# teofum/platinum

Measured on AMD Instinct MI355X. Metric: Msamples/s (paths x spp x bounces / s) at 1920x1080, 8 bounces, higher is better.
Workload: dtype f32; 1 GPU; C3 1.04M-triangle instanced sphere field, 1920x1080; width=1920, height=1080, max_bounces=8, samples_in_flight=128, spp_per_gpu=1792, spp_total=1792, integrator=MIS+NEE, flags=MultiscatterGGX, triangles=1036300, call_pattern=render(spp_per_step) per step, batches=14, nonfinite_policy=zero (a NaN/inf sample counts as black; parity default is propagate), parallelism=sample-sharded x1, one process per GPU + RCCL all-reduce

## Files before the change

### platinum_amd/csrc/kernels.hip

```cpp
#include <hip/hip_runtime.h>

#include "kernels.h"
#include "pt_denoise.h"
#include "pt_post.h"
#include "pt_shade.h"
#include "queue_plan.h"

namespace pt {

__device__ __forceinline__ vec4 ld_stream(const vec4* p) {
  using f4 = __attribute__((ext_vector_type(4))) float;
  const f4 v = __builtin_nontemporal_load((const f4*)p);
  return vec4{v.x, v.y, v.z, v.w};
}
__device__ __forceinline__ uint32_t ld_stream(const uint32_t* p) { return __builtin_nontemporal_load(p); }
__device__ __forceinline__ void st_stream(vec4* p, vec4 v) {
  using f4 = __attribute__((ext_vector_type(4))) float;
  __builtin_nontemporal_store(f4{v.x, v.y, v.z, v.w}, (f4*)p);
}
__device__ __forceinline__ void st_stream(uint32_t* p, uint32_t v) { __builtin_nontemporal_store(v, p); }

__device__ __forceinline__ uint32_t wave_prefix(unsigned long long mask) {
  return __builtin_amdgcn_mbcnt_hi((uint32_t)(mask >> 32), __builtin_amdgcn_mbcnt_lo((uint32_t)mask, 0u));
}
__device__ __forceinline__ uint32_t wave_sum(uint32_t v) {
  for (int off = 32; off > 0; off >>= 1) v += __shfl_xor(v, off, 64);
  return v;
}
__device__ __forceinline__ uint32_t wave_index() { return blockIdx.x * (blockDim.x >> 6) + (threadIdx.x >> 6); }
__device__ __forceinline__ uint32_t wave_count() { return gridDim.x * (blockDim.x >> 6); }
#ifdef PT_TAIL_PROBE
#define PT_TAIL_BEGIN const unsigned long long tail_t0 = wall_clock64(); unsigned long long tail_take = 0, tail_setup = 0, tail_ta = 0;
#define PT_TAIL_T(acc) { const unsigned long long tb_ = wall_clock64(); acc += tb_ - tail_ta; tail_ta = tb_; }
#define PT_TAIL_MARK tail_ta = wall_clock64();
#define PT_TAIL_END(kind)                                                                                         \
  if (wave_lane() == 0 && bounce < 16u) {                                                                           \
    const unsigned long long t1 = wall_clock64();                                                                   \
    atomicMax(&ctr->tail_end_max[kind][bounce], t1); atomicAdd(&ctr->tail_end_sum[kind][bounce], t1);              \
    atomicMax(&ctr->tail_start_inv[kind][bounce], ~tail_t0); atomicAdd(&ctr->tail_waves[kind][bounce], 1ull);     \
    atomicAdd(&ctr->tail_take[kind][bounce], tail_take); atomicAdd(&ctr->tail_setup[kind][bounce], tail_setup);     \
    atomicAdd(&ctr->tail_busy[kind][bounce], t1 - tail_t0);                                                         \
  }
#else
#define PT_TAIL_BEGIN
#define PT_TAIL_END(kind)
#define PT_TAIL_T(acc)
#define PT_TAIL_MARK
#endif

constexpr uint32_t kClaimMax = 8;

__device__ __forceinline__ uint32_t chunk_entry(uint32_t sg, uint32_t k, uint32_t rays) { return ((rays - 1u) << 26) | (k << 16) | sg; }
static_assert(kMaxSegments <= 65536 && kMaxSegmentSlots / 64 <= 1024, "chunk_entry packs 16 + 10 + 6 bits");

struct ChunkClaims {
  const uint32_t* __restrict__ table;
  uint32_t* cursor;
  uint32_t nseg, total, lane;
  uint32_t next_c, end_c, run_c = 0;
  uint32_t e0 = 0, e1 = 0, e2 = 0, e3 = 0, e4 = 0, e5 = 0, e6 = 0, e7 = 0;
  uint32_t claim_k = kClaimMax, nwaves_grid = 1;
  __device__ __forceinline__ void init(const uint32_t* tab, uint32_t total_, uint32_t* cur, const Segments& seg, uint32_t lane_) {
    table = tab; total = total_; cursor = cur; nseg = seg.nseg; lane = lane_;
    next_c = end_c = 0;
    nwaves_grid = gridDim.x * (blockDim.x >> 6);
    claim_k = guided(total);
  }
  __device__ __forceinline__ uint32_t guided(uint32_t remaining) const {
    return remaining > 32u * nwaves_grid ? kClaimMax : remaining > 8u * nwaves_grid ? 4u : remaining > 2u * nwaves_grid ? 2u : 1u;
  }
  uint32_t pool_next = 0, pool_end = 0;
  bool exhausted = false;
  __device__ __forceinline__ uint32_t take(bool need) {
    uint32_t got = kInvalidRef;
    for (;;) {
      const unsigned long long m = __ballot(need && got == kInvalidRef);
      if (m == 0) return got;
      if (pool_next == pool_end) {
        if (exhausted) return got;
        if (next_c == end_c) {
          uint32_t base = 0;
          if (lane == 0) base = atomicAdd(cursor, claim_k);
          base = __builtin_amdgcn_readfirstlane(base);
          if (base >= total) { exhausted = true; return got; }
          next_c = run_c = base;
          end_c = base + claim_k < total ? base + claim_k : total;
          claim_k = guided(total - end_c);
          const int ev = (int)table[base + (lane & 7u)];
          e0 = (uint32_t)__builtin_amdgcn_readlane(ev, 0); e1 = (uint32_t)__builtin_amdgcn_readlane(ev, 1); e2 = (uint32_t)__builtin_amdgcn_readlane(ev, 2);
          e3 = (uint32_t)__builtin_amdgcn_readlane(ev, 3); e4 = (uint32_t)__builtin_amdgcn_readlane(ev, 4); e5 = (uint32_t)__builtin_amdgcn_readlane(ev, 5);
          e6 = (uint32_t)__builtin_amdgcn_readlane(ev, 6); e7 = (uint32_t)__builtin_amdgcn_readlane(ev, 7);
        }
        const uint32_t at = next_c++ - run_c;
        const uint32_t e = at == 0u ? e0 : at == 1u ? e1 : at == 2u ? e2 : at == 3u ? e3 : at == 4u ? e4 : at == 5u ? e5 : at == 6u ? e6 : e7;
        pool_next = seg_slot(nseg, e & 0xffffu, ((e >> 16) & 0x3ffu) * 64u);
        pool_end = pool_next + (e >> 26) + 1u;
      }
      if (need && got == kInvalidRef) {
        const uint32_t idx = pool_next + wave_prefix(m);
        if (idx < pool_end) got = idx;
      }
      const uint32_t avail = pool_end - pool_next, want = (uint32_t)__popcll(m);
      pool_next += want < avail ? want : avail;
    }
  }
};

constexpr uint32_t kTableBlocks = 32;
__global__ void __launch_bounds__(1024) k_chunk_tables(Segments seg, uint32_t cur, BatchCounters* __restrict__ ctr,
                                                        uint32_t bounce_closest, uint32_t bounce_shadow, uint32_t do_shadow) {
  if (blockIdx.y == 2) {
    if (blockIdx.x != 0) return;
    const uint32_t* __restrict__ cnt = seg.active[cur];
    const uint32_t* __restrict__ cost = seg.shade_cost + (size_t)bounce_closest * seg.nseg;
    __shared__ uint32_t hist[256];
    if (threadIdx.x < 256) hist[threadIdx.x] = 0;
    __syncthreads();
    auto size_class = [&](uint32_t w) {
      const uint32_t c = cost[w], v = c ? c : cnt[w];
      const uint32_t e = 31u - (uint32_t)__builtin_clz(v | 8u);
      return 255u - (v < 8u ? v : (e - 2u) * 8u + ((v >> (e - 3u)) & 7u));
    };
    for (uint32_t w = threadIdx.x; w < seg.nseg; w += 1024) atomicAdd(&hist[size_class(w)], 1u);
    __syncthreads();
    if (threadIdx.x == 0) { uint32_t run = 0; for (int b = 0; b < 256; b++) { const uint32_t h = hist[b]; hist[b] = run; run += h; } }
    __syncthreads();
    for (uint32_t w = threadIdx.x; w < seg.nseg; w += 1024) seg.shade_order[atomicAdd(&hist[size_class(w)], 1u)] = w;
    return;
  }
  const bool sh = blockIdx.y == 1;
  if (sh && !do_shadow) return;
  const uint32_t* __restrict__ counts = sh ? seg.shadow : seg.active[cur];
  uint32_t* __restrict__ table = sh ? seg.table_shadow : seg.table_closest;
  __shared__ uint32_t part[1024];
  __shared__ uint32_t base_sh;
  const uint32_t slice = (seg.nseg + kTableBlocks - 1) / kTableBlocks;
  const uint32_t w_begin = blockIdx.x * slice;
  const uint32_t w_end = w_begin + slice < seg.nseg ? w_begin + slice : seg.nseg;
  uint32_t before = 0, total = 0;
  for (uint32_t w = threadIdx.x; w < seg.nseg; w += 1024) {
    const uint32_t nc = (counts[w] + 63u) / 64u;
    total += nc;
    if (w < w_begin) before += nc;
  }
  part[threadIdx.x] = before;
  __syncthreads();
  for (uint32_t off = 512; off > 0; off >>= 1) { if (threadIdx.x < off) part[threadIdx.x] += part[threadIdx.x + off]; __syncthreads(); }
  if (threadIdx.x == 0) base_sh = part[0];
  __syncthreads();
  if (blockIdx.x == kTableBlocks - 1) {
    part[threadIdx.x] = total;
    __syncthreads();
    for (uint32_t off = 512; off > 0; off >>= 1) { if (threadIdx.x < off) part[threadIdx.x] += part[threadIdx.x + off]; __syncthreads(); }
    if (threadIdx.x == 0) {
      if (sh) ctr->chunks_shadow[bounce_shadow] = part[0];
      else ctr->chunks_closest[bounce_closest] = part[0];
    }
    __syncthreads();
  }
  __shared__ uint32_t rays_of[1024];
  const uint32_t mine_n = (w_begin + threadIdx.x < w_end) ? counts[w_begin + threadIdx.x] : 0u;
  rays_of[threadIdx.x] = mine_n;
  const uint32_t mine = (mine_n + 63u) / 64u;
  part[threadIdx.x] = mine;
  __syncthreads();
  for (uint32_t off = 1; off < 1024; off <<= 1) {
    const uint32_t v = threadIdx.x >= off ? part[threadIdx.x - off] : 0;
    __syncthreads();
    part[threadIdx.x] += v;
    __syncthreads();
  }
  const uint32_t n_entries = part[1023];
  const uint32_t base = base_sh;
  for (uint32_t e = threadIdx.x; e < n_entries; e += 1024) {
    uint32_t lo = 0, hi = 1023;
    while (lo < hi) { const uint32_t mid = (lo + hi) >> 1; if (part[mid] > e) hi = mid; else lo = mid + 1; }
    const uint32_t k = e - (lo ? part[lo - 1] : 0u);
    const uint32_t left = rays_of[lo] - k * 64u;
    table[base + e] = chunk_entry(w_begin + lo, k, left < 64u ? left : 64u);
  }
}

__global__ void __launch_bounds__(kBlock) k_raygen(DeviceScene S, PathState st, vec4* __restrict__ Lbuf, Segments seg,
                                                    BatchCounters* __restrict__ ctr, uint32_t first_sample,
                                                    uint32_t nsamples, uint32_t tilesX, uint32_t tilesY) {
  const uint32_t lane = wave_lane();
  const uint32_t tiles = tilesX * tilesY;
  uint32_t started = 0;
  for (uint32_t sg = wave_index(); sg < seg.nseg; sg += wave_count()) {
    uint32_t n_out = 0;
    const uint32_t first_tile = segment_first_tile(seg, sg);
    for (uint32_t k = 0; k < seg.tiles_per_seg * nsamples; k++) {
      const uint32_t tile = first_tile + k / nsamples;
      if (tile >= tiles) break;
      const uint32_t r = (k % nsamples) * 64u + lane;
      const uint32_t pl = r / nsamples, s = r - pl * nsamples;
      const PixelXY q = tile_pixel(tile, pl, tilesX);
      const bool valid = q.x < S.width && q.y < S.height;
      RayGenOut rg;
      if (valid) rg = stage_raygen(S, q.x, q.y, first_sample + s);
      const unsigned long long m = __ballot(valid);
      if (valid) {
        const uint32_t j = seg_slot(seg.nseg, sg, n_out + wave_prefix(m));
        const uint32_t pid = lbuf_index(tile, s, nsamples, pl);
        const uint32_t rel = pid - first_tile * nsamples * 64u;
        st.rayO[j] = vec4{rg.o.x, rg.o.y, rg.o.z, 0.0f};
        st.rayD[j] = vec4{rg.d.x, rg.d.y, rg.d.z, u2f((rg.dim & kMetaDimMask) | (rel << kMetaPidShift))};
        st.att[j] = vec4{1.0f, 1.0f, 1.0f, u2f(rg.offset)};
        Lbuf[pid] = vec4{0.0f, 0.0f, 0.0f, 1.0f};
      }
      n_out += (uint32_t)__popcll(m);
    }
    if (lane == 0) { seg.active[0][sg] = n_out; seg.poison[sg] = 0u; }
    started += n_out;
  }
  if (lane == 0) {
    WaveStats& ws = seg.stats[wave_index()];
    ws.paths += started;
    ws.closest += started;
  }
}

__global__ void __launch_bounds__(kBlock) k_raygen_adaptive(DeviceScene S, PathState st, vec4* __restrict__ Lbuf, Segments seg,
                                                             uint32_t first_sample, uint32_t nsamples, uint32_t tilesX, Rect rect,
                                                             const uint32_t* __restrict__ active, const uint32_t* __restrict__ active_count) {
  const uint32_t lane = wave_lane();
  const uint32_t tiles = *active_count;
  uint32_t started = 0;
  for (uint32_t sg = wave_index(); sg < seg.nseg; sg += wave_count()) {
    uint32_t n_out = 0;
    const uint32_t first_tile = segment_first_tile(seg, sg);
    for (uint32_t k = 0; k < seg.tiles_per_seg * nsamples; k++) {
      const uint32_t tile = first_tile + k / nsamples;
      if (tile >= tiles) break;
      const uint32_t r = (k % nsamples) * 64u + lane;
      const uint32_t pl = r / nsamples, s = r - pl * nsamples;
      const PixelXY q = tile_pixel(active[tile], pl, tilesX);
      const bool valid = rect_contains(rect, q.x, q.y);
      RayGenOut rg;
      if (valid) rg = stage_raygen(S, q.x, q.y, first_sample + s);
      const unsigned long long m = __ballot(valid);
      if (valid) {
        const uint32_t j = seg_slot(seg.nseg, sg, n_out + wave_prefix(m));
        const uint32_t pid = lbuf_index(tile, s, nsamples, pl);
        const uint32_t rel = pid - first_tile * nsamples * 64u;
        st.rayO[j] = vec4{rg.o.x, rg.o.y, rg.o.z, 0.0f};
        st.rayD[j] = vec4{rg.d.x, rg.d.y, rg.d.z, u2f((rg.dim & kMetaDimMask) | (rel << kMetaPidShift))};
        st.att[j] = vec4{1.0f, 1.0f, 1.0f, u2f(rg.offset)};
        Lbuf[pid] = vec4{0.0f, 0.0f, 0.0f, 1.0f};
      }
      n_out += (uint32_t)__popcll(m);
    }
    if (lane == 0) { seg.active[0][sg] = n_out; seg.poison[sg] = 0u; }
    started += n_out;
  }
  if (lane == 0) {
    WaveStats& ws = seg.stats[wave_index()];
    ws.paths += started;
    ws.closest += started;
  }
}

#ifndef PT_TWO_BLOCK
#define PT_TWO_BLOCK 1024
#define PT_TWO_BLOCKS_PER_CU 1
#define PT_TWO_LDS_NODES 1024
#endif
constexpr uint32_t kTraceBlock2 = PT_TWO_BLOCK;
constexpr uint32_t kLdsNodes = PT_TWO_LDS_NODES;
#ifndef PT_TRI_VOTE
#define PT_TRI_VOTE 2
#endif
template <bool ANY, bool COUNT, bool TWO, bool W6 = false>
__device__ __forceinline__ void wave_traverse(const DeviceScene& S, const BvhNode* lds_nodes, TravState& ts, TraversalCount* tc) {
  constexpr int kRoom = W6 ? 1 : 4, kRows = W6 ? kPendLeaves6 : kPendLeaves;
  if (ts.cur != kInvalidRef && ts.st.npend <= kRows - kRoom) {
    if (TWO) {
      trav_leave(ts);
      const bool at_inst = ts.cur != kInvalidRef && (ts.cur & kInstBit) != 0;
      const bool at_node = ts.cur != kInvalidRef && !at_inst;
      const unsigned long long mi = __ballot(at_inst), mn = __ballot(at_node);
      if (mi != 0 && (2 * __popcll(mi) >= __popcll(mn) || mn == 0)) {
        if (at_inst) trav_resolve(S, ts);
      } else if (at_node) {
        if (lds_nodes) trav_node<COUNT, true>(lds_nodes, ts, tc); else trav_node<COUNT, true>(S.nodes, ts, tc);
      }
    } else if (W6) {
      trav_node6<COUNT>(S.nodes, ts, tc);
    } else {
      trav_node<COUNT, false>(S.nodes, ts, tc);
    }
  }
  const bool pending = ts.st.npend > 0;
  const bool stuck = pending && (ts.cur == kInvalidRef || ts.st.npend > kRows - kRoom);
  const bool advancing = ts.cur != kInvalidRef && !stuck;
  const unsigned long long mp = __ballot(pending);
  if (mp == 0) return;
  const bool go = PT_TRI_VOTE * __popcll(mp) >= __popcll(__ballot(1)) || __ballot(ts.st.npend > kRows - kRoom) != 0 || __ballot(advancing) == 0;
  if (go && pending) {
    const bool fin = W6 ? trav_pending_leaf6<ANY, COUNT>(S, ts, tc) : trav_pending_leaf<ANY, COUNT>(S, ts, tc);
    if (fin) { ts.cur = kInvalidRef; ts.st.npend = 0; ts.st.sp = 0; }
  }
}

__device__ __forceinline__ const BvhNode* stage_nodes(const DeviceScene& S, BvhNode* lds_nodes) {
  if (S.node_count > kLdsNodes) return nullptr;
  const uint4* src = reinterpret_cast<const uint4*>(S.nodes);
  uint4* dst = reinterpret_cast<uint4*>(lds_nodes);
  for (uint32_t i = threadIdx.x; i < S.node_count * 4; i += blockDim.x) dst[i] = src[i];
  __syncthreads();
  return lds_nodes;
}

template <bool COUNT, bool TWO, bool W6 = false>
__global__ void __launch_bounds__(TWO ? kTraceBlock2 : kBlock, TWO ? PT_TWO_BLOCKS_PER_CU : PT_CLOSEST_WAVES)
k_trace_closest(DeviceScene S, PathState st, vec4* __restrict__ hit, Segments seg, uint32_t cur, BatchCounters* __restrict__ ctr, uint32_t bounce,
                uint32_t* __restrict__ spill, int32_t* __restrict__ hitlog, uint32_t log_stride) {
  PT_TAIL_BEGIN
  constexpr uint32_t kTB = TWO ? kTraceBlock2 : kBlock;
  __shared__ uint32_t lds_stack[(W6 ? kLdsStack6 : kLdsStack) + 1][kTB];
  __shared__ uint32_t lds_pend[(W6 ? kPendLeaves6 : kPendLeaves) + 1][kTB];
  __shared__ BvhNode lds_nodes_buf[TWO && kLdsNodes ? kLdsNodes : 1];
  const BvhNode* lds_nodes = TWO && kLdsNodes ? stage_nodes(S, lds_nodes_buf) : nullptr;
  const uint32_t lane = wave_lane();
  ChunkClaims src;
  src.init(seg.table_closest, ctr->chunks_closest[bounce], &ctr->work_closest[bounce], seg, lane);
  TraversalStack stack;
  stack.lds = &lds_stack[0][threadIdx.x];
  stack.pend = &lds_pend[0][threadIdx.x];
  stack.lds_stride = kTB;
  stack.spill = spill + ((size_t)blockIdx.x * kTB + threadIdx.x);
  stack.spill_stride = gridDim.x * kTB;
  TraversalCount tc;

  TravState ts;
  uint32_t ray = kInvalidRef;
  auto finish = [&]() {
    const RayHit& h = ts.best;
#ifdef PT_DEBUG_PID
    if (ts.dbg) printf("dbg finish: t %.9g u %.9g v %.9g tri %u gid %u\n", h.t, h.u, h.v, h.tri, h.gid >> 2);
    ts.dbg = false;
#endif
    hit[ray] = vec4{h.t, h.u, h.v, u2f(h.tri == kInvalidRef ? kInvalidRef : (h.tri | ((h.gid & 3u) << 28)))};
    if (hitlog) {
      const uint32_t pixel = pixel_of_pid_1spp(segment_lbuf_base(seg, slot_segment(seg.nseg, ray)) + (f2u(st.rayD[ray].w) >> kMetaPidShift), S.width);
      int32_t* hl = &hitlog[((size_t)bounce * log_stride + pixel) * 2];
      hl[0] = hl[1] = -1;
      if (h.tri != kInvalidRef) triangle_ids(S, h.tri, &hl[0], &hl[1]);
    }
    ray = kInvalidRef;
  };
  const uint32_t refill = seg.refill_threshold;
  for (;;) {
    PT_TAIL_MARK
    const uint32_t fresh = src.take(ray == kInvalidRef);
    PT_TAIL_T(tail_take)
    if (fresh != kInvalidRef) {
      ray = fresh;
      const vec4 o4 = st.rayO[ray];
      const vec4 d4 = st.rayD[ray];
      float ir = 0.0f;
      if (S.has_alpha) ir = Halton{halton_table(S.halton), f2u(st.att[ray].w), f2u(d4.w) & kMetaDimMask}.sample1d();
#ifdef PT_DEBUG_PID
      ts.dbg = ctr->_pad[1] == bounce + 1u && segment_lbuf_base(seg, slot_segment(seg.nseg, ray)) + (f2u(d4.w) >> kMetaPidShift) == ctr->_pad[0];
      if (ts.dbg) printf("dbg ray slot %u lane %u wave %u o %.9g %.9g %.9g d %.9g %.9g %.9g\n", ray, lane, wave_index(), o4.x, o4.y, o4.z, d4.x, d4.y, d4.z);
#endif
      if (trav_init(S, ts, v3(o4.x, o4.y, o4.z), v3(d4.x, d4.y, d4.z), 1e-3f, kInf, ir, stack, false, COUNT ? &tc : nullptr)) finish();
    }
    PT_TAIL_T(tail_setup)
    if (__ballot(ray != kInvalidRef) == 0) {
      if (src.exhausted && src.pool_next == src.pool_end) break;
      continue;
    }
    while (ray != kInvalidRef) {
      wave_traverse<false, COUNT, TWO, W6>(S, lds_nodes, ts, &tc);
      if (ts.cur == kInvalidRef && ts.st.npend == 0) finish();
      if (refill && !src.exhausted && (uint32_t)__popcll(__ballot(ray != kInvalidRef)) < refill) break;
    }
  }
  if (COUNT) {
    const uint32_t nn = wave_sum(tc.nodes), t = wave_sum(tc.tris);
    if (lane == 0) {
      atomicAdd(&ctr->nodes_closest, (unsigned long long)nn);
      atomicAdd(&ctr->tris_closest, (unsigned long long)t);
    }
  }
  PT_TAIL_END(0)
}

#ifndef PT_SHADE_WAVES
#define PT_SHADE_WAVES 4
#endif
#ifndef PT_SHADE_BLOCK
#define PT_SHADE_BLOCK 256
#endif
constexpr uint32_t kShadeBlock = PT_SHADE_BLOCK;
constexpr uint32_t kShadeHalton = 128;
constexpr uint32_t kShadeLights = 64;
constexpr int kLutE = 128, kLutEavg = 128, kLutEavgMs = 32;
constexpr uint32_t kBinCap = 128;

__global__ void __launch_bounds__(PT_SHADE_BLOCK, (PT_SHADE_WAVES * 4 * 64) / PT_SHADE_BLOCK)
k_shade(const DeviceScene* __restrict__ Sp, PathState sin, PathState sout, const vec4* __restrict__ hit, ShadowQueue sq,
        vec4* __restrict__ Lbuf, Segments seg, uint32_t cur, BatchCounters* __restrict__ ctr, uint32_t bounce) {
  PT_TAIL_BEGIN
  const DeviceScene& S = *Sp;
  __shared__ HaltonEntry lds_halton[kShadeHalton];
  __shared__ LightRec lds_lights[kShadeLights];
  __shared__ float lds_Eavg[kLutEavg];
  __shared__ float lds_EavgMs[kLutEavgMs * kLutEavgMs];
  static_assert(kMaxSegmentSlots <= 65536, "slot numbers inside a segment are binned as uint16_t (queue_plan.h bounds seg_cap)");
  __shared__ uint16_t lds_bins[kShadeBlock / 64][5][kBinCap];
  __shared__ uint32_t lds_bin_tri[kShadeBlock / 64][5][kBinCap];
  const uint32_t halton_base = 5u + 7u * bounce;
  uint32_t halton_count = 11u + 5u * bounce;
  if (halton_base >= (uint32_t)kHaltonDims) halton_count = 0;
  else if (halton_base + halton_count > (uint32_t)kHaltonDims) halton_count = (uint32_t)kHaltonDims - halton_base;
  if (halton_count > kShadeHalton) halton_count = kShadeHalton;
  const bool lights_in_lds = S.lightCount <= kShadeLights;
  {
    const uint4* src = reinterpret_cast<const uint4*>(S.halton + halton_base);
    uint4* dst = reinterpret_cast<uint4*>(lds_halton);
    for (uint32_t i = threadIdx.x; i < halton_count * 2; i += kShadeBlock) dst[i] = ldg(&src[i]);
    if (lights_in_lds) {
      const uint4* ls = reinterpret_cast<const uint4*>(S.light_recs);
      uint4* ld = reinterpret_cast<uint4*>(lds_lights);
      for (uint32_t i = threadIdx.x; i < S.lightCount * (uint32_t)(sizeof(LightRec) / 16); i += kShadeBlock) ld[i] = ldg(&ls[i]);
    }
    for (uint32_t i = threadIdx.x; i < (uint32_t)kLutEavg; i += kShadeBlock) lds_Eavg[i] = ldg(&S.luts.Eavg.d[i]);
    for (uint32_t i = threadIdx.x; i < (uint32_t)(kLutEavgMs * kLutEavgMs); i += kShadeBlock) lds_EavgMs[i] = ldg(&S.luts.EavgMs.d[i]);
  }
  __syncthreads();
  ShadeTables T;
  T.luts.E = Lut{S.luts.E.d, kLutE, kLutE, 1, 0};
  T.luts.Eavg = Lut{lds_Eavg, kLutEavg, 1, 1, 1};
  T.luts.EMs = Lut{S.luts.EMs.d, S.luts.EMs.w, S.luts.EMs.h, S.luts.EMs.depth, 0};
  T.luts.EavgMs = Lut{lds_EavgMs, kLutEavgMs, kLutEavgMs, 1, 1};
  T.luts.ETransIn = Lut{S.luts.ETransIn.d, S.luts.ETransIn.w, S.luts.ETransIn.h, S.luts.ETransIn.depth, 0};
  T.luts.ETransOut = Lut{S.luts.ETransOut.d, S.luts.ETransOut.w, S.luts.ETransOut.h, S.luts.ETransOut.depth, 0};
  T.halton = HaltonTab{S.halton, lds_halton, halton_base, halton_count};
  T.lights = lights_in_lds ? lds_lights : S.light_recs;
  T.light_cdf = S.light_cdf;
  T.lights_lds = lights_in_lds ? 1 : 0;

  const uint32_t lane = wave_lane();
  uint32_t shaded = 0, total_out = 0, total_shadow = 0;
  uint32_t claim = wave_index();
  uint16_t* bin = &lds_bins[threadIdx.x >> 6][0][0];
  uint32_t* bin_tri = &lds_bin_tri[threadIdx.x >> 6][0][0];
  while (claim < seg.nseg) {
    const uint32_t sg = __builtin_amdgcn_readfirstlane(seg.shade_order[claim]);
    const unsigned long long seg_t0 = wall_clock64();
    const uint32_t lbuf_base = segment_lbuf_base(seg, sg);
    const uint32_t n = __builtin_amdgcn_readfirstlane(seg.active[cur][sg]);
    uint32_t n_out = 0, n_shadow = 0;
    const uint32_t seg_poisoned = S.env_texture < 0 ? __builtin_amdgcn_readfirstlane(seg.poison[sg]) : 0u;
    unsigned long long poisoned_now = 0;
    uint32_t cnt0 = 0, cnt1 = 0, cnt2 = 0, cnt3 = 0, cnt4 = 0;
    uint32_t k0 = 0;
    for (;;) {
      while (k0 < n && cnt0 < 64 && cnt1 < 64 && cnt2 < 64 && cnt3 < 64 && cnt4 < 64) {
        const uint32_t k = k0 + lane;
        uint32_t cls = 5;
        uint32_t w = 0;
        if (k < n) {
          w = f2u(hit[seg_slot(seg.nseg, sg, k)].w);
          cls = w == kInvalidRef ? 4u : (w >> 28) & 3u;
          if (w == kInvalidRef && S.env_texture < 0) {
            if (!seg_poisoned) cls = 5u;
            else {
              const vec4 a4 = sin.att[seg_slot(seg.nseg, sg, k)];
              if (!att_poisoned(v3(a4.x, a4.y, a4.z))) cls = 5u;
            }
          }
        }
        const unsigned long long m0 = __ballot(cls == 0), m1 = __ballot(cls == 1), m2 = __ballot(cls == 2), m3 = __ballot(cls == 3),
                                 m4 = __ballot(cls == 4);
        if (cls < 5) {
          const uint32_t at = cls == 0 ? cnt0 + wave_prefix(m0) : cls == 1 ? cnt1 + wave_prefix(m1) : cls == 2 ? cnt2 + wave_prefix(m2)
                            : cls == 3 ? cnt3 + wave_prefix(m3) : cnt4 + wave_prefix(m4);
          bin[cls * kBinCap + at] = (uint16_t)k;
          bin_tri[cls * kBinCap + at] = w & kHitTriMask;
        }
        cnt0 += (uint32_t)__popcll(m0); cnt1 += (uint32_t)__popcll(m1); cnt2 += (uint32_t)__popcll(m2);
        cnt3 += (uint32_t)__popcll(m3); cnt4 += (uint32_t)__popcll(m4);
        k0 += 64;
      }
      uint32_t k = kInvalidRef, tri = 0;
      bool is_miss = false;
      const uint32_t full = cnt0 >= 64 ? 0u : cnt1 >= 64 ? 1u : cnt2 >= 64 ? 2u : cnt3 >= 64 ? 3u : cnt4 >= 64 ? 4u : 5u;
      if (full < 5) {
        uint32_t c = 0;
        if (full == 0) c = cnt0 -= 64; else if (full == 1) c = cnt1 -= 64; else if (full == 2) c = cnt2 -= 64;
        else if (full == 3) c = cnt3 -= 64; else c = cnt4 -= 64;
        k = bin[full * kBinCap + c + lane];
        tri = bin_tri[full * kBinCap + c + lane];
        is_miss = full == 4;
      } else {
        if (cnt0 + cnt1 + cnt2 + cnt3 + cnt4 == 0) break;
        uint32_t taken = 0;
#define PT_TAKE_FROM(c, cnt)                                                                                                   \
        {                                                                                                                      \
          const uint32_t take = cnt < 64 - taken ? cnt : 64 - taken;                                                           \
          if (lane >= taken && lane < taken + take) { k = bin[c * kBinCap + cnt - take + (lane - taken)]; tri = bin_tri[c * kBinCap + cnt - take + (lane - taken)]; is_miss = c == 4; }  \
          cnt -= take;                                                                                                         \
          taken += take;                                                                                                       \
        }
        PT_TAKE_FROM(0, cnt0) PT_TAKE_FROM(1, cnt1) PT_TAKE_FROM(2, cnt2) PT_TAKE_FROM(3, cnt3) PT_TAKE_FROM(4, cnt4)
#undef PT_TAKE_FROM
      }
      const bool has = k != kInvalidRef && !is_miss;
      const uint32_t i = seg_slot(seg.nseg, sg, k != kInvalidRef ? k : 0u);
      if (k != kInvalidRef && is_miss) {
        const vec4 o4 = sin.rayO[i];
        const vec4 d4 = sin.rayD[i];
        const vec4 a4 = sin.att[i];
        const vec3 att = v3(a4.x, a4.y, a4.z);
        const uint32_t mpid = lbuf_base + (f2u(d4.w) >> kMetaPidShift);
        vec4 L = Lbuf[mpid];
        if (S.env_texture >= 0) {
          const vec3 Le = stage_miss(S, v3(d4.x, d4.y, d4.z), att, bounce, o4.w, (f2u(d4.w) & kMetaSpecular) != 0);
          L.x += Le.x; L.y += Le.y; L.z += Le.z;
        }
        L.x += att.x * 0.0f; L.y += att.y * 0.0f; L.z += att.z * 0.0f;
        Lbuf[mpid] = L;
      }
      uint32_t c_shadow = 0, c_alive = 0;
      if (has) {
        const vec4 h4 = ld_stream(&hit[i]);
        const vec4 o4 = ld_stream(&sin.rayO[i]);
        const vec4 d4 = ld_stream(&sin.rayD[i]);
        const vec4 a4 = ld_stream(&sin.att[i]);
        const uint32_t meta = f2u(d4.w);
        const uint32_t pid = lbuf_base + (meta >> kMetaPidShift);
        ShadeIn in;
        in.o = v3(o4.x, o4.y, o4.z);
        in.d = v3(d4.x, d4.y, d4.z);
        in.att = v3(a4.x, a4.y, a4.z);
        in.rayO = &sin.rayO[i];
        in.rayD = &sin.rayD[i];
        in.lastSpecular = (meta & kMetaSpecular) != 0;
        in.offset = f2u(a4.w);
        in.dim = (meta & kMetaDimMask) + 1;
        in.bounce = bounce;
        in.t = h4.x; in.u = h4.y; in.v = h4.z;
        in.tri = tri;
        ShadeGeom g;
        ShadingContext sc;
        shade_geometry(S, in, g, sc);
        const BSDF bsdf(sc, S.flags, T.luts, g.wo);
        uint32_t dim_rr;
        {
          const NeeOut nee = shade_nee(S, T, in, g, sc, bsdf, in.dim + 6);
          dim_rr = nee.dim;
          const unsigned long long m = __ballot(nee.shadow);
          if (nee.shadow) {
            const uint32_t j = seg_slot(seg.nseg, sg, n_shadow + wave_prefix(m));
            st_stream(&sq.o[j], vec4{g.hitPos.x, g.hitPos.y, g.hitPos.z, nee.tmax});
            st_stream(&sq.d[j], vec4{nee.d.x, nee.d.y, nee.d.z, u2f(pid)});
            st_stream(&sq.contrib[j], vec4{nee.contrib.x, nee.contrib.y, nee.contrib.z, nee.payload});
          }
          c_shadow = (uint32_t)__popcll(m);
        }
        const BounceOut bo = shade_bounce(S, T, in, g, sc, bsdf, dim_rr);
        if (bo.has_emitted) {
          vec4 L = Lbuf[pid];
          L.x += bo.emitted.x; L.y += bo.emitted.y; L.z += bo.emitted.z;
          Lbuf[pid] = L;
        }
        const unsigned long long m = __ballot(bo.alive);
        poisoned_now |= __ballot(bo.alive && att_poisoned(bo.next_att));
        if (bo.alive) {
          const uint32_t j = seg_slot(seg.nseg, sg, n_out + wave_prefix(m));
          st_stream(&sout.rayO[j], vec4{g.hitPos.x, g.hitPos.y, g.hitPos.z, bo.next_pdf});
          st_stream(&sout.rayD[j], vec4{bo.next_d.x, bo.next_d.y, bo.next_d.z, u2f((bo.dim & kMetaDimMask) | (bo.next_specular ? kMetaSpecular : 0u) | (meta & ~(kMetaDimMask | kMetaSpecular)))});
          st_stream(&sout.att[j], vec4{bo.next_att.x, bo.next_att.y, bo.next_att.z, u2f(in.offset)});
        }
        c_alive = (uint32_t)__popcll(m);
      }
      const unsigned long long mh = __ballot(has);
      if (mh) {
        const int src = __builtin_ctzll(mh);
        n_shadow += (uint32_t)__builtin_amdgcn_readlane((int)c_shadow, src);
        n_out += (uint32_t)__builtin_amdgcn_readlane((int)c_alive, src);
        shaded += (uint32_t)__popcll(mh);
      }
    }
    if (lane == 0) {
      seg.active[cur ^ 1][sg] = n_out;
      seg.shadow[sg] = n_shadow;
      if (poisoned_now) seg.poison[sg] = 1u;
      seg.shade_cost[(size_t)bounce * seg.nseg + sg] = (uint32_t)(wall_clock64() - seg_t0) + 1u;
    }
    total_out += n_out;
    total_shadow += n_shadow;
    uint32_t next = 0;
    if (lane == 0) next = wave_count() + atomicAdd(&ctr->work_shade[bounce], 1u);
    claim = __builtin_amdgcn_readfirstlane(next);
  }
  if (lane == 0) {
    WaveStats& ws = seg.stats[wave_index()];
    ws.closest += total_out;
    ws.shadow += total_shadow;
    ws.shaded += shaded;
  }
  PT_TAIL_END(1)
}

template <bool COUNT, bool TWO, bool W6 = false>
__global__ void __launch_bounds__(TWO ? kTraceBlock2 : kBlock, TWO ? PT_TWO_BLOCKS_PER_CU : PT_SHADOW_WAVES)
k_trace_shadow(DeviceScene S, ShadowQueue sq, vec4* __restrict__ Lbuf, Segments seg, BatchCounters* __restrict__ ctr, uint32_t bounce,
               uint32_t* __restrict__ spill) {
  PT_TAIL_BEGIN
  constexpr uint32_t kTB = TWO ? kTraceBlock2 : kBlock;
  __shared__ uint32_t lds_stack[(W6 ? kLdsStack6 : kLdsStack) + 1][kTB];
  __shared__ uint32_t lds_pend[(W6 ? kPendLeaves6 : kPendLeaves) + 1][kTB];
  __shared__ BvhNode lds_nodes_buf[TWO && kLdsNodes ? kLdsNodes : 1];
  const BvhNode* lds_nodes = TWO && kLdsNodes ? stage_nodes(S, lds_nodes_buf) : nullptr;
  const uint32_t lane = wave_lane();
  ChunkClaims src;
  src.init(seg.table_shadow, ctr->chunks_shadow[bounce], &ctr->work_shadow[bounce], seg, lane);
  TraversalStack stack;
  stack.lds = &lds_stack[0][threadIdx.x];
  stack.pend = &lds_pend[0][threadIdx.x];
  stack.lds_stride = kTB;
  stack.spill = spill + ((size_t)blockIdx.x * kTB + threadIdx.x);
  stack.spill_stride = gridDim.x * kTB;
  TraversalCount tc;

  TravState ts;
  uint32_t ray = kInvalidRef, pid = 0;
  auto finish = [&]() {
    if (ts.best.tri == kInvalidRef) {
      const vec4 c = sq.contrib[ray];
      vec4 L = Lbuf[pid];
      L.x += c.x; L.y += c.y; L.z += c.z;
      Lbuf[pid] = L;
    }
    ray = kInvalidRef;
  };
  const uint32_t refill = seg.refill_threshold;
  for (;;) {
    PT_TAIL_MARK
    const uint32_t fresh = src.take(ray == kInvalidRef);
    PT_TAIL_T(tail_take)
    if (fresh != kInvalidRef) {
      ray = fresh;
      const vec4 o4 = sq.o[ray];
      const vec4 d4 = sq.d[ray];
      pid = f2u(d4.w);
      const float ir = S.has_alpha ? sq.contrib[ray].w : 0.0f;
      if (trav_init(S, ts, v3(o4.x, o4.y, o4.z), v3(d4.x, d4.y, d4.z), 1e-3f, o4.w, ir, stack, true, COUNT ? &tc : nullptr)) finish();
    }
    PT_TAIL_T(tail_setup)
    if (__ballot(ray != kInvalidRef) == 0) {
      if (src.exhausted && src.pool_next == src.pool_end) break;
      continue;
    }
    while (ray != kInvalidRef) {
      wave_traverse<true, COUNT, TWO, W6>(S, lds_nodes, ts, &tc);
      if (ts.cur == kInvalidRef && ts.st.npend == 0) finish();
      if (refill && !src.exhausted && (uint32_t)__popcll(__ballot(ray != kInvalidRef)) < refill) break;
    }
  }
  if (COUNT) {
    const uint32_t nn = wave_sum(tc.nodes), t = wave_sum(tc.tris);
    if (lane == 0) {
      atomicAdd(&ctr->nodes_shadow, (unsigned long long)nn);
      atomicAdd(&ctr->tris_shadow, (unsigned long long)t);
    }
  }
  PT_TAIL_END(2)
}

template <bool ADAPTIVE>
__device__ __forceinline__ void accumulate_body(vec4* __restrict__ acc, const vec4* __restrict__ Lbuf, uint32_t npixels, uint32_t width,
                                                uint32_t nsamples, uint32_t n0, uint32_t nonfinite_policy, BatchCounters* __restrict__ ctr,
                                                const uint32_t* __restrict__ active, const uint32_t* __restrict__ active_count,
                                                vec2* __restrict__ mom, uint32_t* __restrict__ tile_n, Rect rect) {
  constexpr uint32_t kRow = 9;
  __shared__ vec4 stage[kBlock / 64][64 * kRow];
  const uint32_t lane = wave_lane(), w = threadIdx.x >> 6;
  const uint32_t height = npixels / width, tilesX = tiles_x(width), tiles = ADAPTIVE ? *active_count : tilesX * tiles_y(height);
  const uint32_t tile = blockIdx.x * (kBlock / 64) + w;
  const bool live = tile < tiles;
  const uint32_t itile = ADAPTIVE ? (live ? active[tile] : 0u) : tile;
  const PixelXY q = tile_pixel(itile, lane, tilesX);
  const bool inside = live && (ADAPTIVE ? rect_contains(rect, q.x, q.y) : q.x < width && q.y < height);
  const uint32_t p = q.y * width + q.x;
  vec4 a = inside ? acc[p] : vec4{0.0f, 0.0f, 0.0f, 0.0f};
  vec2 m = ADAPTIVE && inside && mom ? mom[p] : vec2{0.0f, 0.0f};
  for (uint32_t s0 = 0; s0 < nsamples; s0 += 8u) {
    const uint32_t nb = nsamples - s0 < 8u ? nsamples - s0 : 8u;
    __syncthreads();
    if (live) {
#pragma unroll
      for (uint32_t i = 0; i < 8u; i++) {
        const uint32_t px = i * 8u + (lane >> 3), j = lane & 7u;
        if (j < nb) stage[w][px * kRow + j] = ld_stream(&Lbuf[lbuf_index(tile, s0 + j, nsamples, px)]);
      }
    }
    __syncthreads();
    if (inside) {
      for (uint32_t j = 0; j < nb; j++) {
        const vec4 v = stage[w][lane * kRow + j];
        vec3 L = v3(v.x, v.y, v.z);
        if (!(fabsf(L.x) <= 3.0e38f && fabsf(L.y) <= 3.0e38f && fabsf(L.z) <= 3.0e38f)) {
          atomicAdd(&ctr->nonfinite, 1u);
          if (nonfinite_policy == PT_NONFINITE_ZERO) L = v3(0.0f);
        }
        const uint32_t localFrameIdx = n0 + s0 + j;
        if (ADAPTIVE) {
          const float lum = dn_lum(L);
          m = vec2{aov_fold(m.x, lum, localFrameIdx), aov_fold(m.y, lum * lum, localFrameIdx)};
        }
        if (localFrameIdx > 0) {
          L = L + v3(a.x, a.y, a.z) * (float)localFrameIdx;
          L = L / (float)(localFrameIdx + 1);
        }
        a = vec4{L.x, L.y, L.z, 1.0f};
      }
    }
  }
  if (inside) acc[p] = a;
  if (ADAPTIVE) {
    if (inside && mom) mom[p] = m;
    if (live && lane == 0) tile_n[itile] = n0 + nsamples;
  }
}

__global__ void __launch_bounds__(kBlock) k_accumulate(vec4* __restrict__ acc, const vec4* __restrict__ Lbuf,
                                                        uint32_t npixels, uint32_t width, uint32_t nsamples, uint32_t n0,
                                                        uint32_t nonfinite_policy, BatchCounters* __restrict__ ctr) {
  accumulate_body<false>(acc, Lbuf, npixels, width, nsamples, n0, nonfinite_policy, ctr, nullptr, nullptr, nullptr, nullptr, Rect{});
}

__global__ void __launch_bounds__(kBlock) k_accumulate_adaptive(vec4* __restrict__ acc, const vec4* __restrict__ Lbuf,
                                                                 uint32_t npixels, uint32_t width, uint32_t nsamples, uint32_t n0,
                                                                 uint32_t nonfinite_policy, BatchCounters* __restrict__ ctr,
                                                                 const uint32_t* __restrict__ active, const uint32_t* __restrict__ active_count,
                                                                 vec2* __restrict__ mom, uint32_t* __restrict__ tile_n, Rect rect) {
  accumulate_body<true>(acc, Lbuf, npixels, width, nsamples, n0, nonfinite_policy, ctr, active, active_count, mom, tile_n, rect);
}

__global__ void __launch_bounds__(kBlock) k_accumulate_gmon(vec4* __restrict__ buckets, const vec4* __restrict__ Lbuf,
                                                             uint32_t npixels, uint32_t width, uint32_t nsamples, uint32_t n0,
                                                             uint32_t samples_per_bucket, uint32_t gmon_buckets, uint32_t bucket_base,
                                                             uint32_t nonfinite_policy, BatchCounters* __restrict__ ctr) {
  const uint32_t p = blockIdx.x * kBlock + threadIdx.x;
  if (p >= npixels) return;
  const uint32_t l0 = lbuf_index_of_pixel(p, width, 0, nsamples);
  constexpr uint32_t kGroup = 8u;
  vec4 v[kGroup];
  for (uint32_t s = 0; s < nsamples; s++) {
    if (s % kGroup == 0) {
#pragma unroll
      for (uint32_t j = 0; j < kGroup; j++)
        if (s + j < nsamples) v[j] = ld_stream(&Lbuf[l0 + (s + j)]);
    }
    vec4 L4 = v[0];
#pragma unroll
    for (uint32_t j = 1; j < kGroup; j++) if (s % kGroup == j) L4 = v[j];
    vec3 L = v3(L4.x, L4.y, L4.z);
    if (!(fabsf(L.x) <= 3.0e38f && fabsf(L.y) <= 3.0e38f && fabsf(L.z) <= 3.0e38f)) {
      atomicAdd(&ctr->nonfinite, 1u);
      if (nonfinite_policy == PT_NONFINITE_ZERO) L = v3(0.0f);
    }
    const uint32_t f = n0 + s;
    vec4* acc = buckets + (size_t)(f / samples_per_bucket - bucket_base) * npixels;
    const uint32_t localFrameIdx = f / gmon_buckets;
    if (localFrameIdx > 0) {
      const vec4 a = acc[p];
      L = L + v3(a.x, a.y, a.z) * (float)localFrameIdx;
      L = L / (float)(localFrameIdx + 1);
    }
    acc[p] = vec4{L.x, L.y, L.z, 1.0f};
  }
}

__global__ void __launch_bounds__(kBlock) k_gmon(vec4* __restrict__ acc, const vec4* __restrict__ buckets, uint32_t npixels,
                                                  uint32_t nBuckets, float cap) {
  const uint32_t p = blockIdx.x * kBlock + threadIdx.x;
  if (p >= npixels) return;
  const vec3 lw = v3(0.2126f, 0.7152f, 0.0722f);
  vec3 values[32];
  for (uint32_t i = 0; i < nBuckets; i++) {
    const vec4 b = buckets[(size_t)i * npixels + p];
    values[i] = v3(b.x, b.y, b.z);
  }
  for (uint32_t i = nBuckets; i > 1; i--)
    for (uint32_t j = 1; j < i; j++)
      if (dot(values[j], lw) < dot(values[j - 1], lw)) {
        const vec3 temp = values[j - 1];
        values[j - 1] = values[j];
        values[j] = temp;
      }
  vec3 sum = v3(0.0f), weightedSum = v3(0.0f);
  for (uint32_t i = 0; i < nBuckets; i++) {
    sum = sum + values[i];
    weightedSum = weightedSum + (float)(i + 1) * values[i];
  }
  float G = (2.0f * dot(weightedSum, lw)) / ((float)nBuckets * dot(sum, lw)) - (float)(nBuckets + 1) / (float)nBuckets;
  G = fminf(G, cap);
  const float cf = G * (float)(nBuckets / 2);
  const int c = cf > 0.0f ? (int)cf : 0;
  sum = v3(0.0f);
  for (int i = c; i < (int)nBuckets - c; i++) sum = sum + values[i];
  const vec3 color = sum / (float)((int)nBuckets - 2 * c);
  acc[p] = vec4{color.x, color.y, color.z, 1.0f};
}

__global__ void __launch_bounds__(kBlock) k_weighted_add(vec4* __restrict__ out, const vec4* __restrict__ in, float w, uint32_t npixels,
                                                          uint32_t first, uint32_t last) {
  const uint32_t p = blockIdx.x * kBlock + threadIdx.x;
  if (p >= npixels) return;
  const vec4 a = in[p];
  vec4 o = first ? vec4{0.0f, 0.0f, 0.0f, 0.0f} : out[p];
  o.x += w * a.x; o.y += w * a.y; o.z += w * a.z;
  o.w = last ? 1.0f : 0.0f;
  out[p] = o;
}

__global__ void __launch_bounds__(kBlock) k_postprocess(const vec4* __restrict__ acc, uint32_t* __restrict__ rgba8, uint32_t W,
                                                         uint32_t H, PostConstants pc) {
  const uint32_t p = blockIdx.x * kBlock + threadIdx.x;
  if (p >= W * H) return;
  const uint32_t py = p / W, px = p - py * W;
  rgba8[p] = pp_pack_rgba8(postprocess_pixel(acc, W, H, px, py, pc));
}

__global__ void __launch_bounds__(kBlock) k_fold_counters(const BatchCounters* __restrict__ ctr, Totals* __restrict__ tot,
                                                           Segments seg, uint32_t counted) {
  __shared__ unsigned long long red[4][kBlock];
  unsigned long long a[4] = {0, 0, 0, 0};
  for (uint32_t w = threadIdx.x; w < seg.nstats; w += kBlock) {
    WaveStats& ws = seg.stats[w];
    a[0] += ws.closest; a[1] += ws.shadow; a[2] += ws.shaded; a[3] += ws.paths;
    ws.closest = 0; ws.shadow = 0; ws.shaded = 0; ws.paths = 0;
  }
  for (int k = 0; k < 4; k++) red[k][threadIdx.x] = a[k];
  __syncthreads();
  if (threadIdx.x != 0) return;
  unsigned long long t[4] = {0, 0, 0, 0};
  for (int k = 0; k < 4; k++)
    for (int i = 0; i < kBlock; i++) t[k] += red[k][i];
  if (!counted) {
    tot->closest_rays += t[0];
    tot->shadow_rays += t[1];
    tot->shaded_hits += t[2];
    tot->paths += t[3];
    tot->nonfinite += ctr->nonfinite;
  } else {
    tot->nodes_closest += ctr->nodes_closest; tot->tris_closest += ctr->tris_closest;
    tot->nodes_shadow += ctr->nodes_shadow; tot->tris_shadow += ctr->tris_shadow;
    tot->counted_closest += t[0]; tot->counted_shadow += t[1];
  }
}

__global__ void __launch_bounds__(kBlock) k_light_records(DeviceScene S, LightRec* __restrict__ out, float* __restrict__ cdf) {
  const uint32_t i = blockIdx.x * kBlock + threadIdx.x;
  if (i < S.lightCount) { out[i] = make_light_rec(S, S.lights[i]); cdf[i] = S.lights[i].cumulativePower; }
}

__global__ void __launch_bounds__(kBlock) k_shade_records(DeviceScene S, ShadeRec* __restrict__ out) {
  const uint32_t t = blockIdx.x * kBlock + threadIdx.x;
  if (t >= 2u * S.slot_count) return;
  const TriRec& tr = S.tris[t >> 1];
  const uint32_t gid = (t & 1u) ? tr.gid_b : tr.gid_a;
  if (gid == kInvalidRef) { out[t] = ShadeRec{}; return; }
  const uint32_t inst = tr.inst_code & kSlotInstMask;
  out[t] = make_shade_rec(S, inst, (gid >> 2) - S.instances[inst].tri_global_base);
}

__global__ void __launch_bounds__(kBlock) k_hit_records(DeviceScene S, PathState st, const vec4* __restrict__ hit, Segments seg,
                                                         pt_hit_record* __restrict__ out) {
  const uint32_t lane = wave_lane();
  for (uint32_t sg = wave_index(); sg < seg.nseg; sg += wave_count()) {
    const uint32_t n = seg.active[0][sg];
    for (uint32_t k = lane; k < n; k += 64) {
      const uint32_t i = seg_slot(seg.nseg, sg, k);
      const vec4 h = hit[i];
      const uint32_t tri = f2u(h.w) == kInvalidRef ? kInvalidRef : (f2u(h.w) & kHitTriMask);
      pt_hit_record r;
      if (tri != kInvalidRef) {
        r.t = h.x; r.u = h.y; r.v = h.z;
        triangle_ids(S, tri, &r.instance, &r.primitive);
      } else {
        r.t = 0.0f; r.u = 0.0f; r.v = 0.0f; r.instance = -1; r.primitive = -1;
      }
      out[pixel_of_pid_1spp(segment_lbuf_base(seg, sg) + (f2u(st.rayD[i].w) >> kMetaPidShift), S.width)] = r;
    }
  }
}

void launch_raygen(hipStream_t s, uint32_t grid, const DeviceScene& S, PathState st, vec4* Lbuf, Segments seg, BatchCounters* ctr,
                   uint32_t first_sample, uint32_t nsamples) {
  hipLaunchKernelGGL(k_raygen, dim3(grid), dim3(kBlock), 0, s, S, st, Lbuf, seg, ctr, first_sample, nsamples, tiles_x(S.width), tiles_y(S.height));
}
void launch_raygen_adaptive(hipStream_t s, uint32_t grid, const DeviceScene& S, PathState st, vec4* Lbuf, Segments seg,
                            uint32_t first_sample, uint32_t nsamples, const Rect& rect, const uint32_t* active, const uint32_t* active_count) {
  hipLaunchKernelGGL(k_raygen_adaptive, dim3(grid), dim3(kBlock), 0, s, S, st, Lbuf, seg, first_sample, nsamples, tiles_x(S.width), rect, active,
                     active_count);
}
void launch_chunk_tables(hipStream_t s, Segments seg, uint32_t cur, BatchCounters* ctr, uint32_t bounce_closest,
                         uint32_t bounce_shadow, bool do_shadow) {
  hipLaunchKernelGGL(k_chunk_tables, dim3(kTableBlocks, 3), dim3(1024), 0, s, seg, cur, ctr, bounce_closest, bounce_shadow, do_shadow ? 1u : 0u);
}
uint32_t trace_block_threads(bool two_level) { return two_level ? kTraceBlock2 : (uint32_t)kBlock; }
uint32_t trace_blocks_per_cu_two_level() { return PT_TWO_BLOCKS_PER_CU; }
void launch_trace_closest(hipStream_t s, uint32_t grid, const DeviceScene& S, PathState st, vec4* hit, Segments seg, uint32_t cur,
                          BatchCounters* ctr, uint32_t bounce, uint32_t* spill, int32_t* hitlog, uint32_t log_stride, bool count) {
  if (S.two_level) {
    if (count)
      hipLaunchKernelGGL((k_trace_closest<true, true>), dim3(grid), dim3(kTraceBlock2), 0, s, S, st, hit, seg, cur, ctr, bounce, spill, hitlog, log_stride);
    else
      hipLaunchKernelGGL((k_trace_closest<false, true>), dim3(grid), dim3(kTraceBlock2), 0, s, S, st, hit, seg, cur, ctr, bounce, spill, hitlog, log_stride);
    return;
  }
  if (S.wide6) {
    if (count)
      hipLaunchKernelGGL((k_trace_closest<true, false, true>), dim3(grid), dim3(kBlock), 0, s, S, st, hit, seg, cur, ctr, bounce, spill, hitlog, log_stride);
    else
      hipLaunchKernelGGL((k_trace_closest<false, false, true>), dim3(grid), dim3(kBlock), 0, s, S, st, hit, seg, cur, ctr, bounce, spill, hitlog, log_stride);
    return;
  }
  if (count)
    hipLaunchKernelGGL((k_trace_closest<true, false>), dim3(grid), dim3(kBlock), 0, s, S, st, hit, seg, cur, ctr, bounce, spill, hitlog, log_stride);
  else
    hipLaunchKernelGGL((k_trace_closest<false, false>), dim3(grid), dim3(kBlock), 0, s, S, st, hit, seg, cur, ctr, bounce, spill, hitlog, log_stride);
}
uint32_t shade_block_threads() { return kShadeBlock; }
uint32_t shade_blocks_per_cu() { return (PT_SHADE_WAVES * 4 * 64) / PT_SHADE_BLOCK; }
void launch_shade(hipStream_t s, uint32_t grid, const DeviceScene* S, PathState sin, PathState sout, const vec4* hit,
                  ShadowQueue sq, vec4* Lbuf, Segments seg, uint32_t cur, BatchCounters* ctr, uint32_t bounce) {
  hipLaunchKernelGGL(k_shade, dim3(grid), dim3(kShadeBlock), 0, s, S, sin, sout, hit, sq, Lbuf, seg, cur, ctr, bounce);
}
void launch_trace_shadow(hipStream_t s, uint32_t grid, const DeviceScene& S, ShadowQueue sq, vec4* Lbuf, Segments seg,
                         BatchCounters* ctr, uint32_t bounce, uint32_t* spill, bool count) {
  if (S.two_level) {
    if (count) hipLaunchKernelGGL((k_trace_shadow<true, true>), dim3(grid), dim3(kTraceBlock2), 0, s, S, sq, Lbuf, seg, ctr, bounce, spill);
    else hipLaunchKernelGGL((k_trace_shadow<false, true>), dim3(grid), dim3(kTraceBlock2), 0, s, S, sq, Lbuf, seg, ctr, bounce, spill);
    return;
  }
  if (S.wide6) {
    if (count) hipLaunchKernelGGL((k_trace_shadow<true, false, true>), dim3(grid), dim3(kBlock), 0, s, S, sq, Lbuf, seg, ctr, bounce, spill);
    else hipLaunchKernelGGL((k_trace_shadow<false, false, true>), dim3(grid), dim3(kBlock), 0, s, S, sq, Lbuf, seg, ctr, bounce, spill);
    return;
  }
  if (count) hipLaunchKernelGGL((k_trace_shadow<true, false>), dim3(grid), dim3(kBlock), 0, s, S, sq, Lbuf, seg, ctr, bounce, spill);
  else hipLaunchKernelGGL((k_trace_shadow<false, false>), dim3(grid), dim3(kBlock), 0, s, S, sq, Lbuf, seg, ctr, bounce, spill);
}
void launch_accumulate(hipStream_t s, vec4* acc, const vec4* Lbuf, uint32_t npixels, uint32_t width, uint32_t nsamples, uint32_t n0,
                       uint32_t nonfinite_policy, BatchCounters* ctr) {
  const uint32_t tiles = tile_count(width, npixels / width);
  hipLaunchKernelGGL(k_accumulate, dim3((tiles + kBlock / 64 - 1) / (kBlock / 64)), dim3(kBlock), 0, s, acc, Lbuf, npixels, width, nsamples, n0,
                     nonfinite_policy, ctr);
}
void launch_accumulate_adaptive(hipStream_t s, vec4* acc, const vec4* Lbuf, uint32_t npixels, uint32_t width, uint32_t nsamples, uint32_t n0,
                                uint32_t nonfinite_policy, BatchCounters* ctr, const uint32_t* active, const uint32_t* active_count,
                                uint32_t max_active, vec2* mom, uint32_t* tile_n, const Rect& rect) {
  const uint32_t tiles = max_active;
  hipLaunchKernelGGL(k_accumulate_adaptive, dim3((tiles + kBlock / 64 - 1) / (kBlock / 64)), dim3(kBlock), 0, s, acc, Lbuf, npixels, width, nsamples,
                     n0, nonfinite_policy, ctr, active, active_count, mom, tile_n, rect);
}
void launch_accumulate_gmon(hipStream_t s, vec4* buckets, const vec4* Lbuf, uint32_t npixels, uint32_t width, uint32_t nsamples, uint32_t n0,
                            uint32_t samples_per_bucket, uint32_t gmon_buckets, uint32_t bucket_base, uint32_t nonfinite_policy, BatchCounters* ctr) {
  hipLaunchKernelGGL(k_accumulate_gmon, dim3((npixels + kBlock - 1) / kBlock), dim3(kBlock), 0, s, buckets, Lbuf, npixels, width, nsamples, n0,
                     samples_per_bucket, gmon_buckets, bucket_base, nonfinite_policy, ctr);
}
void launch_weighted_add(hipStream_t s, vec4* out, const vec4* in, float w, uint32_t npixels, bool first, bool last) {
  hipLaunchKernelGGL(k_weighted_add, dim3((npixels + kBlock - 1) / kBlock), dim3(kBlock), 0, s, out, in, w, npixels, first ? 1u : 0u, last ? 1u : 0u);
}
void launch_gmon(hipStream_t s, vec4* acc, const vec4* buckets, uint32_t npixels, uint32_t nBuckets, float cap) {
  hipLaunchKernelGGL(k_gmon, dim3((npixels + kBlock - 1) / kBlock), dim3(kBlock), 0, s, acc, buckets, npixels, nBuckets, cap);
}
void launch_postprocess(hipStream_t s, const vec4* acc, uint32_t* rgba8, uint32_t W, uint32_t H, const PostConstants& pc) {
  hipLaunchKernelGGL(k_postprocess, dim3((W * H + kBlock - 1) / kBlock), dim3(kBlock), 0, s, acc, rgba8, W, H, pc);
}
void launch_fold_counters(hipStream_t s, const BatchCounters* ctr, Totals* tot, Segments seg, bool counted) {
  hipLaunchKernelGGL(k_fold_counters, dim3(1), dim3(kBlock), 0, s, ctr, tot, seg, counted ? 1u : 0u);
}
void launch_shade_records(hipStream_t s, const DeviceScene& S, ShadeRec* out) {
  if (S.slot_count) hipLaunchKernelGGL(k_shade_records, dim3((2u * S.slot_count + kBlock - 1) / kBlock), dim3(kBlock), 0, s, S, out);
}
void launch_light_records(hipStream_t s, const DeviceScene& S, LightRec* out, float* cdf) {
  if (S.lightCount) hipLaunchKernelGGL(k_light_records, dim3((S.lightCount + kBlock - 1) / kBlock), dim3(kBlock), 0, s, S, out, cdf);
}
void launch_hit_records(hipStream_t s, uint32_t grid, const DeviceScene& S, PathState st, const vec4* hit, Segments seg,
                        pt_hit_record* out) {
  hipLaunchKernelGGL(k_hit_records, dim3(grid), dim3(kBlock), 0, s, S, st, hit, seg, out);
}

}
```

### platinum_amd/csrc/pt_shade.h

```cpp
#pragma once
#include "pt_bvh.h"

namespace pt {

struct Frame {
  vec3 x, y, z;
  PT_HD vec3 worldToLocal(vec3 w) const { return {dot(w, x), dot(w, y), dot(w, z)}; }
  PT_HD vec3 localToWorld(vec3 l) const { return (x * l.x + y * l.y) + z * l.z; }
};
PT_HD Frame frame_from_normal(vec3 n) {
  const vec3 a = fabsf(n.x) > 0.5f ? v3(0.0f, 0.0f, 1.0f) : v3(1.0f, 0.0f, 0.0f);
  const vec3 b = normalize(cross(n, a));
  const vec3 t = cross(n, b);
  return {t, b, n};
}
PT_HD Frame frame_from_nt(vec3 n, vec3 t, float sgn) {
  if (fabsf(dot(n, t)) > 0.9f) return frame_from_normal(n);
  const vec3 b = normalize(cross(n, t)) * sgn;
  t = cross(b, n);
  return {t, b, n};
}

struct Xform { vec3 c0, c1, c2, c3; };
PT_HD Xform load_xform(const InstanceInfo& in) {
  return {v3(in.c0[0], in.c0[1], in.c0[2]), v3(in.c1[0], in.c1[1], in.c1[2]), v3(in.c2[0], in.c2[1], in.c2[2]),
          v3(in.c3[0], in.c3[1], in.c3[2])};
}
PT_HD vec3 transformVec(vec3 p, const Xform& m) { return (m.c0 * p.x + m.c1 * p.y) + m.c2 * p.z; }
PT_HD vec3 transformPoint(vec3 p, const Xform& m) { return ((m.c0 * p.x + m.c1 * p.y) + m.c2 * p.z) + m.c3; }
PT_HD vec3 ld3(const pt_float3& v) { return v3(v.x, v.y, v.z); }

PT_HD vec3 interpolate3(vec3 a0, vec3 a1, vec3 a2, float u, float v) { return ((1.0f - u - v) * a0 + u * a1) + v * a2; }

PT_HD uint32_t material_class(const pt_material_gpu& m) {
  if (m.clearcoat > 0.0f || m.clearcoatTextureId >= 0 || m.rmTextureId >= 0 || m.transmissionTextureId >= 0) return 3u;
  if (m.transmission > 0.0f) return 2u;
  if (m.metallic > 0.0f) return 1u;
  return 0u;
}

PT_HD ShadeRec make_shade_rec(const DeviceScene& S, uint32_t instanceIdx, uint32_t prim) {
  const InstanceInfo& inst = S.instances[instanceIdx];
  const MeshInfo mesh = S.meshes[inst.mesh];
  const uint32_t* __restrict__ idx = &S.indices[3 * (size_t)(mesh.tri_base + prim)];
  ShadeRec r;
  r.v[0] = mesh.vertex_base + idx[0]; r.v[1] = mesh.vertex_base + idx[1]; r.v[2] = mesh.vertex_base + idx[2];
  r.material = inst.material_base + S.slots[mesh.tri_base + prim];
  r.inst = instanceIdx;
  const vec3 p0 = ld3(S.positions[r.v[0]]), p1 = ld3(S.positions[r.v[1]]), p2 = ld3(S.positions[r.v[2]]);
  const vec3 geometricNormal = normalize(cross(p1 - p0, p2 - p0));
  const vec3 ws = normalize(transformVec(geometricNormal, load_xform(inst)));
  r.ng[0] = ws.x; r.ng[1] = ws.y; r.ng[2] = ws.z;
  return r;
}

PT_HD LightRec make_light_rec(const DeviceScene& S, const pt_area_light& light) {
  const InstanceInfo& linst = S.instances[light.instanceIdx];
  const uint32_t vb = S.meshes[linst.mesh].vertex_base;
  const vec3 q0 = ld3(S.positions[vb + light.indices[0]]);
  const vec3 q1 = ld3(S.positions[vb + light.indices[1]]);
  const vec3 q2 = ld3(S.positions[vb + light.indices[2]]);
  const vec3 osNormal = cross(q1 - q0, q2 - q0);
  const vec3 n = normalize(transformVec(osNormal, load_xform(linst)));
  LightRec r;
  r.q0[0] = q0.x; r.q0[1] = q0.y; r.q0[2] = q0.z; r.area = light.area;
  r.q1[0] = q1.x; r.q1[1] = q1.y; r.q1[2] = q1.z; r.power = light.power;
  r.q2[0] = q2.x; r.q2[1] = q2.y; r.q2[2] = q2.z; r.cumulativePower = light.cumulativePower;
  for (int k = 0; k < 3; k++) { r.c0[k] = linst.c0[k]; r.c1[k] = linst.c1[k]; r.c2[k] = linst.c2[k]; r.c3[k] = linst.c3[k]; }
  r.e0 = light.emission.x; r.e1 = light.emission.y; r.e2 = light.emission.z;
  r.n[0] = n.x; r.n[1] = n.y; r.n[2] = n.z;
  r._pad0 = 0.0f; r._pad1 = 0.0f;
  return r;
}

struct RayGenOut { vec3 o, d; uint32_t offset, dim; };

PT_HD RayGenOut stage_raygen(const DeviceScene& S, uint32_t px, uint32_t py, uint32_t sample) {
  Halton h{halton_table(S.halton), halton_offset(px, py, sample), 0};
  const vec2 pixelSample = h.sample2d();
  vec2 lensSample = {0.0f, 0.0f};
  if (S.camera.apertureRadius > 0.0f) lensSample = h.sample2d(); else h.dim += 2;
  const pt_camera_data& cam = S.camera;
  vec3 origin = ld3(cam.position);
  if (cam.apertureRadius > 0.0f) {
    vec2 lensPos = sampleDiskPolar(lensSample);
    lensPos.x = powr_det(lensPos.x, exp2_det(cam.bokehPower));
    if (cam.apertureRoundness < 1.0f) {
      const float n = (float)cam.apertureBlades;
      const float rPolygon = cos_det(kPi / n) / cos_det(fmodf(lensPos.y + 1.5f * kPi, 2.0f * kPi / n) - kPi / n);
      const float r = mix(rPolygon, 1.0f, cam.apertureRoundness);
      lensPos.x = lensPos.x * r;
    }
    float s, c;
    sincos_det(lensPos.y, &s, &c);
    const float lx = lensPos.x * c * cam.apertureRadius;
    const float ly = lensPos.x * s * cam.apertureRadius;
    origin = origin + (lx * normalize(ld3(cam.pixelDeltaU)) + ly * normalize(ld3(cam.pixelDeltaV)));
  }
  const float fx = (float)px + pixelSample.x;
  const float fy = (float)py + pixelSample.y;
  RayGenOut out;
  out.o = origin;
  out.d = normalize(((ld3(cam.topLeft) + fx * ld3(cam.pixelDeltaU)) + fy * ld3(cam.pixelDeltaV)) - origin);
  out.offset = h.offset;
  out.dim = h.dim;
  return out;
}

struct ShadeIn {
  vec3 o, d;
  vec3 att;
  const vec4* rayO;
  const vec4* rayD;
  bool lastSpecular;
  uint32_t offset, dim;
  uint32_t bounce;
  float t, u, v;
  uint32_t tri;
};
struct ShadeOut {
  vec3 emitted;
  bool has_emitted;
  bool shadow;
  vec3 shadow_o, shadow_d;
  float shadow_tmax;
  vec3 shadow_contrib;
  float shadow_payload;
  bool alive;
  vec3 next_o, next_d, next_att;
  float next_pdf;
  bool next_specular;
  uint32_t dim;
};

struct ShadeTables {
  LutSet luts;
  HaltonTab halton;
  const LightRec* lights;
  const float* light_cdf;
  int lights_lds;
};
PT_HD ShadeTables shade_tables(const DeviceScene& S) { return {S.luts, halton_table(S.halton), S.light_recs, S.light_cdf, 0}; }
PT_HD LightRec load_light(const ShadeTables& T, uint32_t i) { return T.lights_lds ? T.lights[i] : ldg(&T.lights[i]); }
PT_HD float light_cumulative_power(const ShadeTables& T, uint32_t i) {
  return T.lights_lds ? T.lights[i].cumulativePower : ldg(&T.light_cdf[i]);
}

PT_HD vec2 rayDirToUv(vec3 dir) {
  const float phi = atan2_det(-dir.z, -dir.x);
  const float theta = acos_det(dir.y);
  return {phi / (2.0f * kPi), theta / kPi};
}
PT_HD vec3 uvToRayDir(vec2 uv) {
  float y, r, cosPhi, sinPhi;
  sincos_det(uv.y * kPi, &r, &y);
  sincos_det(uv.x * 2.0f * kPi, &sinPhi, &cosPhi);
  return normalize(v3(-cosPhi * r, y, -sinPhi * r));
}

struct EnvSample { vec3 Li, wi; float pdf; };
PT_HD EnvSample sample_environment(const DeviceScene& S, vec2 r) {
  const TexInfo t = ldg(&S.textures[S.env_texture]);
  const uint64_t w = t.w, h = t.h, n = w * h;
  uint64_t i = (uint64_t)(r.x * (float)n);
  if (i > n - 1) i = n - 1;
  if (r.y >= ldg(&S.env_alias[i].p)) i = ldg(&S.env_alias[i].aliasIdx);
  const uint64_t x = i % w, y = i / w;
  const vec2 uv = {(float)x / (float)w, (float)y / (float)h};
  const vec4 Le = tex_sample(S, S.env_texture, uv);
  EnvSample es;
  es.Li = v3(Le.x, Le.y, Le.z);
  es.wi = uvToRayDir(uv);
  es.pdf = ldg(&S.env_alias[i].pdf) / (4.0f * kPi);
  return es;
}

PT_HD vec3 stage_miss(const DeviceScene& S, vec3 d, vec3 att, uint32_t bounce, float lastPdf, bool lastSpecular) {
  const TexInfo t = ldg(&S.textures[S.env_texture]);
  const vec2 uv = rayDirToUv(d);
  const vec4 s = tex_sample(S, S.env_texture, uv);
  const vec3 Le = v3(s.x, s.y, s.z);
  if (S.integrator != PT_INTEGRATOR_MIS || bounce == 0 || lastSpecular) return att * Le;
  const float fxw = (float)t.w * uv.x, fyh = (float)t.h * uv.y;
  uint32_t x = fxw > 0.0f ? (uint32_t)fxw : 0u, y = fyh > 0.0f ? (uint32_t)fyh : 0u;
  x = x < t.w - 1 ? x : t.w - 1;
  y = y < t.h - 1 ? y : t.h - 1;
  const float lightPdf = ldg(&S.env_alias[(size_t)y * t.w + x].pdf) * 0.25f * 0.318309886183790671538f;
  const float bsdfWeight = lastPdf / (lastPdf + lightPdf);
  return att * bsdfWeight * Le;
}

PT_HD uint32_t sampleLightPower(const DeviceScene& S, const ShadeTables& T, float r) {
  r = r * S.totalLightPower;
  uint32_t sz = S.lightCount - 1, idx = 0u;
  while (sz > 0) {
    const uint32_t h = sz >> 1, middle = idx + h;
    const bool res = light_cumulative_power(T, middle) < r;
    idx = res ? (middle + 1) : idx;
    sz = res ? sz - (h + 1) : h;
  }
  return idx > S.lightCount - 1 ? S.lightCount - 1 : idx;
}


struct ShadeGeom {
  vec3 hitPos;
  Frame frame;
  vec3 wo;
};
PT_HD void shade_geometry(const DeviceScene& S, const ShadeIn& in, ShadeGeom& g, ShadingContext& ctx) {
  const ShadeRec rec = ldg(&S.shade_recs[in.tri]);
  const InstanceInfo inst = ldg(&S.instances[rec.inst]);
  const pt_material_gpu material = ldg(&S.materials[rec.material]);
  const pt_vertex_data vd0 = ldg(&S.vdata[rec.v[0]]), vd1 = ldg(&S.vdata[rec.v[1]]), vd2 = ldg(&S.vdata[rec.v[2]]);
  const float tangentSign = vd0.tangent[3];

  const vec3 surfaceNormal = interpolate3(ld3(vd0.normal), ld3(vd1.normal), ld3(vd2.normal), in.u, in.v);
  const vec3 surfaceTangent = interpolate3(v3(vd0.tangent[0], vd0.tangent[1], vd0.tangent[2]),
                                           v3(vd1.tangent[0], vd1.tangent[1], vd1.tangent[2]),
                                           v3(vd2.tangent[0], vd2.tangent[1], vd2.tangent[2]), in.u, in.v);
  const float wb = 1.0f - in.u - in.v;
  const vec2 surfaceUV = {(wb * vd0.texCoords[0] + in.u * vd1.texCoords[0]) + in.v * vd2.texCoords[0],
                          (wb * vd0.texCoords[1] + in.u * vd1.texCoords[1]) + in.v * vd2.texCoords[1]};

  const Xform objectToWorld = load_xform(inst);
  g.hitPos = in.o + in.d * in.t;
  const vec3 wsSurfaceNormal = normalize(transformVec(surfaceNormal, objectToWorld));
  const vec3 wsSurfaceTangent = normalize(transformVec(surfaceTangent, objectToWorld));
  g.frame = frame_from_nt(wsSurfaceNormal, wsSurfaceTangent, tangentSign);
  if (material.normalTextureId >= 0) {
    const vec4 t = tex_sample(S, material.normalTextureId, surfaceUV);
    const vec3 sampledNormal = v3(t.x, t.y, t.z) * 2.0f - v3(1.0f);
    g.frame = frame_from_normal(g.frame.localToWorld(sampledNormal));
  }
  g.wo = g.frame.worldToLocal(-in.d);
  ctx = make_shading_context(S, material, surfaceUV);
}

struct NeeOut {
  bool shadow;
  vec3 d;
  float tmax;
  vec3 contrib;
  float payload;
  uint32_t dim;
};
PT_HD NeeOut shade_nee(const DeviceScene& S, const ShadeTables& T, const ShadeIn& in, const ShadeGeom& g, const ShadingContext& ctx,
                       const BSDF& bsdf, uint32_t dim) {
  NeeOut out;
  out.shadow = false;
  out.dim = dim;
  if (!(S.integrator == PT_INTEGRATOR_MIS && (ctx.roughness > 0.0f || ctx.metallic + ctx.transmission < 1.0f))) return out;
  Halton halton{T.halton, in.offset, dim};
  const vec2 rl = halton.sample2d();
  float rz = halton.sample1d();
  out.dim = halton.dim;
  const uint32_t envCount = S.envLightCount;
  if (!(S.lightCount > 0 || envCount > 0)) return out;
  const float pInfinite = S.lightCount == 0 ? 1.0f : (float)envCount / (float)(envCount + 1);
  vec3 Li, lpos, lwi;
  float lpdf, pLight;
  if (rz < pInfinite) {
    rz = rz / pInfinite;
    pLight = pInfinite / (float)envCount;
    const EnvSample es = sample_environment(S, rl);
    Li = es.Li; lpos = es.wi * 100.0f; lwi = es.wi; lpdf = es.pdf;
  } else {
    rz = (rz - pInfinite) / (1.0f - pInfinite);
    const LightRec light = load_light(T, sampleLightPower(S, T, rz));
    pLight = (1.0f - pInfinite) * light.power / S.totalLightPower;
    const vec3 q0 = v3(light.q0[0], light.q0[1], light.q0[2]), q1 = v3(light.q1[0], light.q1[1], light.q1[2]),
               q2 = v3(light.q2[0], light.q2[1], light.q2[2]);
    const vec2 sc = sampleTriUniform(rl);
    const Xform lx = {v3(light.c0[0], light.c0[1], light.c0[2]), v3(light.c1[0], light.c1[1], light.c1[2]),
                      v3(light.c2[0], light.c2[1], light.c2[2]), v3(light.c3[0], light.c3[1], light.c3[2])};
    lpos = transformPoint(interpolate3(q0, q1, q2, sc.x, sc.y), lx);
    const vec3 lnormal = v3(light.n[0], light.n[1], light.n[2]);
    lwi = normalize(lpos - g.hitPos);
    lpdf = length_squared(lpos - g.hitPos) / (fabsf(dot(lnormal, lwi)) * light.area);
    Li = v3(light.e0, light.e1, light.e2);
  }

  const vec3 wi = g.frame.worldToLocal(lwi);
  const BsdfEval ev = bsdf.eval(g.wo, wi);
  if (length_squared(ev.f) > 0.0f) {
    out.payload = S.has_alpha ? halton.sample1d() : (halton.dim++, 0.0f);
    out.dim = halton.dim;
    const float pdfLight = pLight * lpdf;
    const vec3 Ld = Li * ev.f * fabsf(wi.z) / (pdfLight + ev.pdf);
    out.shadow = true;
    out.d = lwi;
    out.tmax = length(lpos - g.hitPos) - 1e-3f;
    out.contrib = in.att * Ld;
  }
  return out;
}

struct BounceOut {
  vec3 emitted;
  bool has_emitted;
  bool alive;
  vec3 next_d, next_att;
  float next_pdf;
  bool next_specular;
  uint32_t dim;
};
PT_HD bool att_poisoned(vec3 a) { return !(fabsf(a.x) <= 3.0e38f && fabsf(a.y) <= 3.0e38f && fabsf(a.z) <= 3.0e38f); }
PT_HD BounceOut shade_bounce(const DeviceScene& S, const ShadeTables& T, const ShadeIn& in, const ShadeGeom& g, const ShadingContext& ctx,
                             const BSDF& bsdf, uint32_t dim_rr) {
  BounceOut out;
  out.has_emitted = false;
  out.alive = false;
  out.emitted = v3(0.0f);
  const bool mis = S.integrator == PT_INTEGRATOR_MIS;
  Halton halton{T.halton, in.offset, in.dim};
  const vec2 r01 = halton.sample2d();
  const float r2 = halton.sample1d();
  float r3 = 0.0f;
  {
    const float m = ctx.metallic, pT = m + (1.0f - m) * ctx.transmission;
    if (ctx.clearcoat > 0.0f || (m > 0.0f && m < 1.0f) || (pT > 0.0f && pT < 1.0f)) r3 = halton.sample1d(); else halton.dim += 1;
  }
  vec2 rc = {0.0f, 0.0f};
  if (ctx.clearcoat > 0.0f) rc = halton.sample2d(); else halton.dim += 2;
  const BsdfSample sample = bsdf.sample(g.wo, vec4{r01.x, r01.y, r2, r3}, rc);

  if (sample.flags & Sample_Emitted) {
    out.has_emitted = true;
    if (!mis || in.bounce == 0 || in.lastSpecular) {
      out.emitted = in.att * sample.Le;
    } else {
      const ShadeRec rec = ldg(&S.shade_recs[in.tri]);
      const vec3 wsGeometricNormal = v3(rec.ng[0], rec.ng[1], rec.ng[2]);
      const vec4 o4 = ldg(in.rayO), d4 = ldg(in.rayD);
      const vec3 ro = v3(o4.x, o4.y, o4.z), rd = v3(d4.x, d4.y, d4.z);
      const float lastPdf = o4.w;
      const float lightPdf = (sample.Le.y * kPi / S.totalLightPower) * length_squared(ro - g.hitPos) /
                             fabsf(dot(rd, wsGeometricNormal));
      const float bsdfWeight = lastPdf / (lastPdf + lightPdf);
      out.emitted = in.att * bsdfWeight * sample.Le;
    }
  }

  halton.dim = dim_rr;
  out.dim = halton.dim;
  if (!(sample.flags & (Sample_Reflected | Sample_Transmitted))) return out;

  vec3 att = in.att * (sample.f * fabsf(sample.wi.z) / sample.pdf);
  if (in.bounce > 0) {
    const float q = fmaxf(0.0f, 1.0f - fmaxf(att.x, fmaxf(att.y, att.z)));
    if (q > 0.0f) {
      if (halton.sample1d() < q) { out.dim = halton.dim; return out; }
    } else halton.dim += 1;
    att = att / (1.0f - q);
  }
  out.dim = halton.dim;
  if (in.bounce + 1 >= S.max_bounces) return out;

  out.alive = true;
  out.next_d = normalize(g.frame.localToWorld(sample.wi));
  out.next_att = att;
  out.next_pdf = sample.pdf;
  out.next_specular = (sample.flags & Sample_Specular) != 0;
  return out;
}

PT_HD ShadeOut stage_shade(const DeviceScene& S, const ShadeIn& in) {
  const ShadeTables T = shade_tables(S);
  ShadeGeom g;
  ShadingContext ctx;
  shade_geometry(S, in, g, ctx);
  const BSDF bsdf(ctx, S.flags, T.luts, g.wo);
  const NeeOut nee = shade_nee(S, T, in, g, ctx, bsdf, in.dim + 6);
  const BounceOut bo = shade_bounce(S, T, in, g, ctx, bsdf, nee.dim);
  ShadeOut out;
  out.emitted = bo.emitted;
  out.has_emitted = bo.has_emitted;
  out.shadow = nee.shadow;
  out.shadow_o = g.hitPos;
  out.shadow_d = nee.shadow ? nee.d : v3(0.0f);
  out.shadow_tmax = nee.shadow ? nee.tmax : 0.0f;
  out.shadow_contrib = nee.shadow ? nee.contrib : v3(0.0f);
  out.shadow_payload = nee.shadow ? nee.payload : 0.0f;
  out.alive = bo.alive;
  out.next_o = g.hitPos;
  out.next_d = bo.alive ? bo.next_d : v3(0.0f);
  out.next_att = bo.alive ? bo.next_att : v3(0.0f);
  out.next_pdf = bo.alive ? bo.next_pdf : 0.0f;
  out.next_specular = bo.alive ? bo.next_specular : false;
  out.dim = bo.dim;
  return out;
}

}
```

Baseline: 9500 Msamples/s.

## Park shade-kernel per-lane state in LDS to cut register pressure

Moves the shade kernel into its own file and stores long-lived per-lane values (attenuation, offset, hit position, metadata, slot index) in LDS instead of registers across the NEE and bounce stages. They are reloaded through a `parked()` accessor at the point of use. Shadow counts also go through LDS with an opaque zero to force a scalar read. The goal is fewer live VGPRs and so higher occupancy or less spilling, at the cost of extra LDS traffic and footprint.

```diff
diff --git a/platinum_amd/csrc/kernels.hip b/platinum_amd/csrc/kernels.hip
--- a/platinum_amd/csrc/kernels.hip
+++ b/platinum_amd/csrc/kernels.hip
@@ -1,6 +1,7 @@
 #include <hip/hip_runtime.h>
 
 #include "kernels.h"
+#include "kernels_wave.h"
 #include "pt_denoise.h"
 #include "pt_post.h"
 #include "pt_shade.h"
@@ -8,45 +9,6 @@
 
 namespace pt {
 
-__device__ __forceinline__ vec4 ld_stream(const vec4* p) {
-  using f4 = __attribute__((ext_vector_type(4))) float;
-  const f4 v = __builtin_nontemporal_load((const f4*)p);
-  return vec4{v.x, v.y, v.z, v.w};
-}
-__device__ __forceinline__ uint32_t ld_stream(const uint32_t* p) { return __builtin_nontemporal_load(p); }
-__device__ __forceinline__ void st_stream(vec4* p, vec4 v) {
-  using f4 = __attribute__((ext_vector_type(4))) float;
-  __builtin_nontemporal_store(f4{v.x, v.y, v.z, v.w}, (f4*)p);
-}
-__device__ __forceinline__ void st_stream(uint32_t* p, uint32_t v) { __builtin_nontemporal_store(v, p); }
-
-__device__ __forceinline__ uint32_t wave_prefix(unsigned long long mask) {
-  return __builtin_amdgcn_mbcnt_hi((uint32_t)(mask >> 32), __builtin_amdgcn_mbcnt_lo((uint32_t)mask, 0u));
-}
-__device__ __forceinline__ uint32_t wave_sum(uint32_t v) {
-  for (int off = 32; off > 0; off >>= 1) v += __shfl_xor(v, off, 64);
-  return v;
-}
-__device__ __forceinline__ uint32_t wave_index() { return blockIdx.x * (blockDim.x >> 6) + (threadIdx.x >> 6); }
-__device__ __forceinline__ uint32_t wave_count() { return gridDim.x * (blockDim.x >> 6); }
-#ifdef PT_TAIL_PROBE
-#define PT_TAIL_BEGIN const unsigned long long tail_t0 = wall_clock64(); unsigned long long tail_take = 0, tail_setup = 0, tail_ta = 0;
-#define PT_TAIL_T(acc) { const unsigned long long tb_ = wall_clock64(); acc += tb_ - tail_ta; tail_ta = tb_; }
-#define PT_TAIL_MARK tail_ta = wall_clock64();
-#define PT_TAIL_END(kind)                                                                                         \
-  if (wave_lane() == 0 && bounce < 16u) {                                                                           \
-    const unsigned long long t1 = wall_clock64();                                                                   \
-    atomicMax(&ctr->tail_end_max[kind][bounce], t1); atomicAdd(&ctr->tail_end_sum[kind][bounce], t1);              \
-    atomicMax(&ctr->tail_start_inv[kind][bounce], ~tail_t0); atomicAdd(&ctr->tail_waves[kind][bounce], 1ull);     \
-    atomicAdd(&ctr->tail_take[kind][bounce], tail_take); atomicAdd(&ctr->tail_setup[kind][bounce], tail_setup);     \
-    atomicAdd(&ctr->tail_busy[kind][bounce], t1 - tail_t0);                                                         \
-  }
-#else
-#define PT_TAIL_BEGIN
-#define PT_TAIL_END(kind)
-#define PT_TAIL_T(acc)
-#define PT_TAIL_MARK
-#endif
 
 constexpr uint32_t kClaimMax = 8;
 
@@ -388,224 +350,6 @@
   PT_TAIL_END(0)
 }
 
-#ifndef PT_SHADE_WAVES
-#define PT_SHADE_WAVES 4
-#endif
-#ifndef PT_SHADE_BLOCK
-#define PT_SHADE_BLOCK 256
-#endif
-constexpr uint32_t kShadeBlock = PT_SHADE_BLOCK;
-constexpr uint32_t kShadeHalton = 128;
-constexpr uint32_t kShadeLights = 64;
-constexpr int kLutE = 128, kLutEavg = 128, kLutEavgMs = 32;
-constexpr uint32_t kBinCap = 128;
-
-__global__ void __launch_bounds__(PT_SHADE_BLOCK, (PT_SHADE_WAVES * 4 * 64) / PT_SHADE_BLOCK)
-k_shade(const DeviceScene* __restrict__ Sp, PathState sin, PathState sout, const vec4* __restrict__ hit, ShadowQueue sq,
-        vec4* __restrict__ Lbuf, Segments seg, uint32_t cur, BatchCounters* __restrict__ ctr, uint32_t bounce) {
-  PT_TAIL_BEGIN
-  const DeviceScene& S = *Sp;
-  __shared__ HaltonEntry lds_halton[kShadeHalton];
-  __shared__ LightRec lds_lights[kShadeLights];
-  __shared__ float lds_Eavg[kLutEavg];
-  __shared__ float lds_EavgMs[kLutEavgMs * kLutEavgMs];
-  static_assert(kMaxSegmentSlots <= 65536, "slot numbers inside a segment are binned as uint16_t (queue_plan.h bounds seg_cap)");
-  __shared__ uint16_t lds_bins[kShadeBlock / 64][5][kBinCap];
-  __shared__ uint32_t lds_bin_tri[kShadeBlock / 64][5][kBinCap];
-  const uint32_t halton_base = 5u + 7u * bounce;
-  uint32_t halton_count = 11u + 5u * bounce;
-  if (halton_base >= (uint32_t)kHaltonDims) halton_count = 0;
-  else if (halton_base + halton_count > (uint32_t)kHaltonDims) halton_count = (uint32_t)kHaltonDims - halton_base;
-  if (halton_count > kShadeHalton) halton_count = kShadeHalton;
-  const bool lights_in_lds = S.lightCount <= kShadeLights;
-  {
-    const uint4* src = reinterpret_cast<const uint4*>(S.halton + halton_base);
-    uint4* dst = reinterpret_cast<uint4*>(lds_halton);
-    for (uint32_t i = threadIdx.x; i < halton_count * 2; i += kShadeBlock) dst[i] = ldg(&src[i]);
-    if (lights_in_lds) {
-      const uint4* ls = reinterpret_cast<const uint4*>(S.light_recs);
-      uint4* ld = reinterpret_cast<uint4*>(lds_lights);
-      for (uint32_t i = threadIdx.x; i < S.lightCount * (uint32_t)(sizeof(LightRec) / 16); i += kShadeBlock) ld[i] = ldg(&ls[i]);
-    }
-    for (uint32_t i = threadIdx.x; i < (uint32_t)kLutEavg; i += kShadeBlock) lds_Eavg[i] = ldg(&S.luts.Eavg.d[i]);
-    for (uint32_t i = threadIdx.x; i < (uint32_t)(kLutEavgMs * kLutEavgMs); i += kShadeBlock) lds_EavgMs[i] = ldg(&S.luts.EavgMs.d[i]);
-  }
-  __syncthreads();
-  ShadeTables T;
-  T.luts.E = Lut{S.luts.E.d, kLutE, kLutE, 1, 0};
-  T.luts.Eavg = Lut{lds_Eavg, kLutEavg, 1, 1, 1};
-  T.luts.EMs = Lut{S.luts.EMs.d, S.luts.EMs.w, S.luts.EMs.h, S.luts.EMs.depth, 0};
-  T.luts.EavgMs = Lut{lds_EavgMs, kLutEavgMs, kLutEavgMs, 1, 1};
-  T.luts.ETransIn = Lut{S.luts.ETransIn.d, S.luts.ETransIn.w, S.luts.ETransIn.h, S.luts.ETransIn.depth, 0};
-  T.luts.ETransOut = Lut{S.luts.ETransOut.d, S.luts.ETransOut.w, S.luts.ETransOut.h, S.luts.ETransOut.depth, 0};
-  T.halton = HaltonTab{S.halton, lds_halton, halton_base, halton_count};
-  T.lights = lights_in_lds ? lds_lights : S.light_recs;
-  T.light_cdf = S.light_cdf;
-  T.lights_lds = lights_in_lds ? 1 : 0;
-
-  const uint32_t lane = wave_lane();
-  uint32_t shaded = 0, total_out = 0, total_shadow = 0;
-  uint32_t claim = wave_index();
-  uint16_t* bin = &lds_bins[threadIdx.x >> 6][0][0];
-  uint32_t* bin_tri = &lds_bin_tri[threadIdx.x >> 6][0][0];
-  while (claim < seg.nseg) {
-    const uint32_t sg = __builtin_amdgcn_readfirstlane(seg.shade_order[claim]);
-    const unsigned long long seg_t0 = wall_clock64();
-    const uint32_t lbuf_base = segment_lbuf_base(seg, sg);
-    const uint32_t n = __builtin_amdgcn_readfirstlane(seg.active[cur][sg]);
-    uint32_t n_out = 0, n_shadow = 0;
-    const uint32_t seg_poisoned = S.env_texture < 0 ? __builtin_amdgcn_readfirstlane(seg.poison[sg]) : 0u;
-    unsigned long long poisoned_now = 0;
-    uint32_t cnt0 = 0, cnt1 = 0, cnt2 = 0, cnt3 = 0, cnt4 = 0;
-    uint32_t k0 = 0;
-    for (;;) {
-      while (k0 < n && cnt0 < 64 && cnt1 < 64 && cnt2 < 64 && cnt3 < 64 && cnt4 < 64) {
-        const uint32_t k = k0 + lane;
-        uint32_t cls = 5;
-        uint32_t w = 0;
-        if (k < n) {
-          w = f2u(hit[seg_slot(seg.nseg, sg, k)].w);
-          cls = w == kInvalidRef ? 4u : (w >> 28) & 3u;
-          if (w == kInvalidRef && S.env_texture < 0) {
-            if (!seg_poisoned) cls = 5u;
-            else {
-              const vec4 a4 = sin.att[seg_slot(seg.nseg, sg, k)];
-              if (!att_poisoned(v3(a4.x, a4.y, a4.z))) cls = 5u;
-            }
-          }
-        }
-        const unsigned long long m0 = __ballot(cls == 0), m1 = __ballot(cls == 1), m2 = __ballot(cls == 2), m3 = __ballot(cls == 3),
-                                 m4 = __ballot(cls == 4);
-        if (cls < 5) {
-          const uint32_t at = cls == 0 ? cnt0 + wave_prefix(m0) : cls == 1 ? cnt1 + wave_prefix(m1) : cls == 2 ? cnt2 + wave_prefix(m2)
-                            : cls == 3 ? cnt3 + wave_prefix(m3) : cnt4 + wave_prefix(m4);
-          bin[cls * kBinCap + at] = (uint16_t)k;
-          bin_tri[cls * kBinCap + at] = w & kHitTriMask;
-        }
-        cnt0 += (uint32_t)__popcll(m0); cnt1 += (uint32_t)__popcll(m1); cnt2 += (uint32_t)__popcll(m2);
-        cnt3 += (uint32_t)__popcll(m3); cnt4 += (uint32_t)__popcll(m4);
-        k0 += 64;
-      }
-      uint32_t k = kInvalidRef, tri = 0;
-      bool is_miss = false;
-      const uint32_t full = cnt0 >= 64 ? 0u : cnt1 >= 64 ? 1u : cnt2 >= 64 ? 2u : cnt3 >= 64 ? 3u : cnt4 >= 64 ? 4u : 5u;
-      if (full < 5) {
-        uint32_t c = 0;
-        if (full == 0) c = cnt0 -= 64; else if (full == 1) c = cnt1 -= 64; else if (full == 2) c = cnt2 -= 64;
-        else if (full == 3) c = cnt3 -= 64; else c = cnt4 -= 64;
-        k = bin[full * kBinCap + c + lane];
-        tri = bin_tri[full * kBinCap + c + lane];
-        is_miss = full == 4;
-      } else {
-        if (cnt0 + cnt1 + cnt2 + cnt3 + cnt4 == 0) break;
-        uint32_t taken = 0;
-#define PT_TAKE_FROM(c, cnt)                                                                                                   \
-        {                                                                                                                      \
-          const uint32_t take = cnt < 64 - taken ? cnt : 64 - taken;                                                           \
-          if (lane >= taken && lane < taken + take) { k = bin[c * kBinCap + cnt - take + (lane - taken)]; tri = bin_tri[c * kBinCap + cnt - take + (lane - taken)]; is_miss = c == 4; }  \
-          cnt -= take;                                                                                                         \
-          taken += take;                                                                                                       \
-        }
-        PT_TAKE_FROM(0, cnt0) PT_TAKE_FROM(1, cnt1) PT_TAKE_FROM(2, cnt2) PT_TAKE_FROM(3, cnt3) PT_TAKE_FROM(4, cnt4)
-#undef PT_TAKE_FROM
-      }
-      const bool has = k != kInvalidRef && !is_miss;
-      const uint32_t i = seg_slot(seg.nseg, sg, k != kInvalidRef ? k : 0u);
-      if (k != kInvalidRef && is_miss) {
-        const vec4 o4 = sin.rayO[i];
-        const vec4 d4 = sin.rayD[i];
-        const vec4 a4 = sin.att[i];
-        const vec3 att = v3(a4.x, a4.y, a4.z);
-        const uint32_t mpid = lbuf_base + (f2u(d4.w) >> kMetaPidShift);
-        vec4 L = Lbuf[mpid];
-        if (S.env_texture >= 0) {
-          const vec3 Le = stage_miss(S, v3(d4.x, d4.y, d4.z), att, bounce, o4.w, (f2u(d4.w) & kMetaSpecular) != 0);
-          L.x += Le.x; L.y += Le.y; L.z += Le.z;
-        }
-        L.x += att.x * 0.0f; L.y += att.y * 0.0f; L.z += att.z * 0.0f;
-        Lbuf[mpid] = L;
-      }
-      uint32_t c_shadow = 0, c_alive = 0;
-      if (has) {
-        const vec4 h4 = ld_stream(&hit[i]);
-        const vec4 o4 = ld_stream(&sin.rayO[i]);
-        const vec4 d4 = ld_stream(&sin.rayD[i]);
-        const vec4 a4 = ld_stream(&sin.att[i]);
-        const uint32_t meta = f2u(d4.w);
-        const uint32_t pid = lbuf_base + (meta >> kMetaPidShift);
-        ShadeIn in;
-        in.o = v3(o4.x, o4.y, o4.z);
-        in.d = v3(d4.x, d4.y, d4.z);
-        in.att = v3(a4.x, a4.y, a4.z);
-        in.rayO = &sin.rayO[i];
-        in.rayD = &sin.rayD[i];
-        in.lastSpecular = (meta & kMetaSpecular) != 0;
-        in.offset = f2u(a4.w);
-        in.dim = (meta & kMetaDimMask) + 1;
-        in.bounce = bounce;
-        in.t = h4.x; in.u = h4.y; in.v = h4.z;
-        in.tri = tri;
-        ShadeGeom g;
-        ShadingContext sc;
-        shade_geometry(S, in, g, sc);
-        const BSDF bsdf(sc, S.flags, T.luts, g.wo);
-        uint32_t dim_rr;
-        {
-          const NeeOut nee = shade_nee(S, T, in, g, sc, bsdf, in.dim + 6);
-          dim_rr = nee.dim;
-          const unsigned long long m = __ballot(nee.shadow);
-          if (nee.shadow) {
-            const uint32_t j = seg_slot(seg.nseg, sg, n_shadow + wave_prefix(m));
-            st_stream(&sq.o[j], vec4{g.hitPos.x, g.hitPos.y, g.hitPos.z, nee.tmax});
-            st_stream(&sq.d[j], vec4{nee.d.x, nee.d.y, nee.d.z, u2f(pid)});
-            st_stream(&sq.contrib[j], vec4{nee.contrib.x, nee.contrib.y, nee.contrib.z, nee.payload});
-          }
-          c_shadow = (uint32_t)__popcll(m);
-        }
-        const BounceOut bo = shade_bounce(S, T, in, g, sc, bsdf, dim_rr);
-        if (bo.has_emitted) {
-          vec4 L = Lbuf[pid];
-          L.x += bo.emitted.x; L.y += bo.emitted.y; L.z += bo.emitted.z;
-          Lbuf[pid] = L;
-        }
-        const unsigned long long m = __ballot(bo.alive);
-        poisoned_now |= __ballot(bo.alive && att_poisoned(bo.next_att));
-        if (bo.alive) {
-          const uint32_t j = seg_slot(seg.nseg, sg, n_out + wave_prefix(m));
-          st_stream(&sout.rayO[j], vec4{g.hitPos.x, g.hitPos.y, g.hitPos.z, bo.next_pdf});
-          st_stream(&sout.rayD[j], vec4{bo.next_d.x, bo.next_d.y, bo.next_d.z, u2f((bo.dim & kMetaDimMask) | (bo.next_specular ? kMetaSpecular : 0u) | (meta & ~(kMetaDimMask | kMetaSpecular)))});
-          st_stream(&sout.att[j], vec4{bo.next_att.x, bo.next_att.y, bo.next_att.z, u2f(in.offset)});
-        }
-        c_alive = (uint32_t)__popcll(m);
-      }
-      const unsigned long long mh = __ballot(has);
-      if (mh) {
-        const int src = __builtin_ctzll(mh);
-        n_shadow += (uint32_t)__builtin_amdgcn_readlane((int)c_shadow, src);
-        n_out += (uint32_t)__builtin_amdgcn_readlane((int)c_alive, src);
-        shaded += (uint32_t)__popcll(mh);
-      }
-    }
-    if (lane == 0) {
-      seg.active[cur ^ 1][sg] = n_out;
-      seg.shadow[sg] = n_shadow;
-      if (poisoned_now) seg.poison[sg] = 1u;
-      seg.shade_cost[(size_t)bounce * seg.nseg + sg] = (uint32_t)(wall_clock64() - seg_t0) + 1u;
-    }
-    total_out += n_out;
-    total_shadow += n_shadow;
-    uint32_t next = 0;
-    if (lane == 0) next = wave_count() + atomicAdd(&ctr->work_shade[bounce], 1u);
-    claim = __builtin_amdgcn_readfirstlane(next);
-  }
-  if (lane == 0) {
-    WaveStats& ws = seg.stats[wave_index()];
-    ws.closest += total_out;
-    ws.shadow += total_shadow;
-    ws.shaded += shaded;
-  }
-  PT_TAIL_END(1)
-}
 
 template <bool COUNT, bool TWO, bool W6 = false>
 __global__ void __launch_bounds__(TWO ? kTraceBlock2 : kBlock, TWO ? PT_TWO_BLOCKS_PER_CU : PT_SHADOW_WAVES)
@@ -929,12 +673,6 @@
   else
     hipLaunchKernelGGL((k_trace_closest<false, false>), dim3(grid), dim3(kBlock), 0, s, S, st, hit, seg, cur, ctr, bounce, spill, hitlog, log_stride);
 }
-uint32_t shade_block_threads() { return kShadeBlock; }
-uint32_t shade_blocks_per_cu() { return (PT_SHADE_WAVES * 4 * 64) / PT_SHADE_BLOCK; }
-void launch_shade(hipStream_t s, uint32_t grid, const DeviceScene* S, PathState sin, PathState sout, const vec4* hit,
-                  ShadowQueue sq, vec4* Lbuf, Segments seg, uint32_t cur, BatchCounters* ctr, uint32_t bounce) {
-  hipLaunchKernelGGL(k_shade, dim3(grid), dim3(kShadeBlock), 0, s, S, sin, sout, hit, sq, Lbuf, seg, cur, ctr, bounce);
-}
 void launch_trace_shadow(hipStream_t s, uint32_t grid, const DeviceScene& S, ShadowQueue sq, vec4* Lbuf, Segments seg,
                          BatchCounters* ctr, uint32_t bounce, uint32_t* spill, bool count) {
   if (S.two_level) {
diff --git a/platinum_amd/csrc/kernels_wave.h b/platinum_amd/csrc/kernels_wave.h
--- /dev/null
+++ b/platinum_amd/csrc/kernels_wave.h
@@ -0,0 +1,48 @@
+#pragma once
+#include <hip/hip_runtime.h>
+
+#include "kernels.h"
+
+namespace pt {
+
+__device__ __forceinline__ vec4 ld_stream(const vec4* p) {
+  using f4 = __attribute__((ext_vector_type(4))) float;
+  const f4 v = __builtin_nontemporal_load((const f4*)p);
+  return vec4{v.x, v.y, v.z, v.w};
+}
+__device__ __forceinline__ uint32_t ld_stream(const uint32_t* p) { return __builtin_nontemporal_load(p); }
+__device__ __forceinline__ void st_stream(vec4* p, vec4 v) {
+  using f4 = __attribute__((ext_vector_type(4))) float;
+  __builtin_nontemporal_store(f4{v.x, v.y, v.z, v.w}, (f4*)p);
+}
+__device__ __forceinline__ void st_stream(uint32_t* p, uint32_t v) { __builtin_nontemporal_store(v, p); }
+
+__device__ __forceinline__ uint32_t wave_prefix(unsigned long long mask) {
+  return __builtin_amdgcn_mbcnt_hi((uint32_t)(mask >> 32), __builtin_amdgcn_mbcnt_lo((uint32_t)mask, 0u));
+}
+__device__ __forceinline__ uint32_t wave_sum(uint32_t v) {
+  for (int off = 32; off > 0; off >>= 1) v += __shfl_xor(v, off, 64);
+  return v;
+}
+__device__ __forceinline__ uint32_t wave_index() { return blockIdx.x * (blockDim.x >> 6) + (threadIdx.x >> 6); }
+__device__ __forceinline__ uint32_t wave_count() { return gridDim.x * (blockDim.x >> 6); }
+#ifdef PT_TAIL_PROBE
+#define PT_TAIL_BEGIN const unsigned long long tail_t0 = wall_clock64(); unsigned long long tail_take = 0, tail_setup = 0, tail_ta = 0;
+#define PT_TAIL_T(acc) { const unsigned long long tb_ = wall_clock64(); acc += tb_ - tail_ta; tail_ta = tb_; }
+#define PT_TAIL_MARK tail_ta = wall_clock64();
+#define PT_TAIL_END(kind)                                                                                         \
+  if (wave_lane() == 0 && bounce < 16u) {                                                                           \
+    const unsigned long long t1 = wall_clock64();                                                                   \
+    atomicMax(&ctr->tail_end_max[kind][bounce], t1); atomicAdd(&ctr->tail_end_sum[kind][bounce], t1);              \
+    atomicMax(&ctr->tail_start_inv[kind][bounce], ~tail_t0); atomicAdd(&ctr->tail_waves[kind][bounce], 1ull);     \
+    atomicAdd(&ctr->tail_take[kind][bounce], tail_take); atomicAdd(&ctr->tail_setup[kind][bounce], tail_setup);     \
+    atomicAdd(&ctr->tail_busy[kind][bounce], t1 - tail_t0);                                                         \
+  }
+#else
+#define PT_TAIL_BEGIN
+#define PT_TAIL_END(kind)
+#define PT_TAIL_T(acc)
+#define PT_TAIL_MARK
+#endif
+
+}
diff --git a/platinum_amd/csrc/pt_shade.h b/platinum_amd/csrc/pt_shade.h
--- a/platinum_amd/csrc/pt_shade.h
+++ b/platinum_amd/csrc/pt_shade.h
@@ -133,6 +133,15 @@
   uint32_t dim;
 };
 
+struct LastRay { vec3 o, d; float pdf, t; uint32_t tri; bool specular; };
+PT_HD vec3 path_att(const ShadeIn& in) { return in.att; }
+PT_HD uint32_t path_offset(const ShadeIn& in) { return in.offset; }
+PT_HD uint32_t path_dim(const ShadeIn& in) { return in.dim; }
+PT_HD LastRay path_last_ray(const ShadeIn& in) {
+  const vec4 o4 = ldg(in.rayO), d4 = ldg(in.rayD);
+  return {v3(o4.x, o4.y, o4.z), v3(d4.x, d4.y, d4.z), o4.w, in.t, in.tri, in.lastSpecular};
+}
+
 struct ShadeTables {
   LutSet luts;
   HaltonTab halton;
@@ -245,13 +254,14 @@
   float payload;
   uint32_t dim;
 };
-PT_HD NeeOut shade_nee(const DeviceScene& S, const ShadeTables& T, const ShadeIn& in, const ShadeGeom& g, const ShadingContext& ctx,
+template <class In>
+PT_HD NeeOut shade_nee(const DeviceScene& S, const ShadeTables& T, const In& in, const ShadeGeom& g, const ShadingContext& ctx,
                        const BSDF& bsdf, uint32_t dim) {
   NeeOut out;
   out.shadow = false;
   out.dim = dim;
   if (!(S.integrator == PT_INTEGRATOR_MIS && (ctx.roughness > 0.0f || ctx.metallic + ctx.transmission < 1.0f))) return out;
-  Halton halton{T.halton, in.offset, dim};
+  Halton halton{T.halton, path_offset(in), dim};
   const vec2 rl = halton.sample2d();
   float rz = halton.sample1d();
   out.dim = halton.dim;
@@ -281,17 +291,18 @@
     Li = v3(light.e0, light.e1, light.e2);
   }
 
+  const float dist = length(lpos - g.hitPos);
+  const float pdfLight = pLight * lpdf;
   const vec3 wi = g.frame.worldToLocal(lwi);
   const BsdfEval ev = bsdf.eval(g.wo, wi);
   if (length_squared(ev.f) > 0.0f) {
     out.payload = S.has_alpha ? halton.sample1d() : (halton.dim++, 0.0f);
     out.dim = halton.dim;
-    const float pdfLight = pLight * lpdf;
     const vec3 Ld = Li * ev.f * fabsf(wi.z) / (pdfLight + ev.pdf);
     out.shadow = true;
     out.d = lwi;
-    out.tmax = length(lpos - g.hitPos) - 1e-3f;
-    out.contrib = in.att * Ld;
+    out.tmax = dist - 1e-3f;
+    out.contrib = path_att(in) * Ld;
   }
   return out;
 }
@@ -306,14 +317,17 @@
   uint32_t dim;
 };
 PT_HD bool att_poisoned(vec3 a) { return !(fabsf(a.x) <= 3.0e38f && fabsf(a.y) <= 3.0e38f && fabsf(a.z) <= 3.0e38f); }
-PT_HD BounceOut shade_bounce(const DeviceScene& S, const ShadeTables& T, const ShadeIn& in, const ShadeGeom& g, const ShadingContext& ctx,
+template <class In>
+PT_HD BounceOut shade_bounce(const DeviceScene& S, const ShadeTables& T, const In& in, const ShadeGeom& g, const ShadingContext& ctx,
                              const BSDF& bsdf, uint32_t dim_rr) {
   BounceOut out;
   out.has_emitted = false;
   out.alive = false;
   out.emitted = v3(0.0f);
+  out.dim = dim_rr;
+  if (in.bounce + 1 >= S.max_bounces && !(ctx.flags & PT_MATERIAL_EMISSIVE)) return out;
   const bool mis = S.integrator == PT_INTEGRATOR_MIS;
-  Halton halton{T.halton, in.offset, in.dim};
+  Halton halton{T.halton, path_offset(in), path_dim(in)};
   const vec2 r01 = halton.sample2d();
   const float r2 = halton.sample1d();
   float r3 = 0.0f;
@@ -327,34 +341,32 @@
 
   if (sample.flags & Sample_Emitted) {
     out.has_emitted = true;
-    if (!mis || in.bounce == 0 || in.lastSpecular) {
-      out.emitted = in.att * sample.Le;
+    const LastRay lr = (mis && in.bounce != 0) ? path_last_ray(in) : LastRay{v3(0.0f), v3(0.0f), 0.0f, 0.0f, 0u, true};
+    if (lr.specular) {
+      out.emitted = path_att(in) * sample.Le;
     } else {
-      const ShadeRec rec = ldg(&S.shade_recs[in.tri]);
+      const ShadeRec rec = ldg(&S.shade_recs[lr.tri]);
       const vec3 wsGeometricNormal = v3(rec.ng[0], rec.ng[1], rec.ng[2]);
-      const vec4 o4 = ldg(in.rayO), d4 = ldg(in.rayD);
-      const vec3 ro = v3(o4.x, o4.y, o4.z), rd = v3(d4.x, d4.y, d4.z);
-      const float lastPdf = o4.w;
-      const float lightPdf = (sample.Le.y * kPi / S.totalLightPower) * length_squared(ro - g.hitPos) /
-                             fabsf(dot(rd, wsGeometricNormal));
-      const float bsdfWeight = lastPdf / (lastPdf + lightPdf);
-      out.emitted = in.att * bsdfWeight * sample.Le;
+      const vec3 hitPos = lr.o + lr.d * lr.t;
+      const float lightPdf = (sample.Le.y * kPi / S.totalLightPower) * length_squared(lr.o - hitPos) /
+                             fabsf(dot(lr.d, wsGeometricNormal));
+      const float bsdfWeight = lr.pdf / (lr.pdf + lightPdf);
+      out.emitted = path_att(in) * bsdfWeight * sample.Le;
     }
   }
 
-  halton.dim = dim_rr;
-  out.dim = halton.dim;
+  out.dim = dim_rr;
   if (!(sample.flags & (Sample_Reflected | Sample_Transmitted))) return out;
 
-  vec3 att = in.att * (sample.f * fabsf(sample.wi.z) / sample.pdf);
+  vec3 att = path_att(in) * (sample.f * fabsf(sample.wi.z) / sample.pdf);
   if (in.bounce > 0) {
     const float q = fmaxf(0.0f, 1.0f - fmaxf(att.x, fmaxf(att.y, att.z)));
     if (q > 0.0f) {
-      if (halton.sample1d() < q) { out.dim = halton.dim; return out; }
-    } else halton.dim += 1;
+      if (Halton{T.halton, path_offset(in), dim_rr}.sample1d() < q) { out.dim = dim_rr + 1; return out; }
+    }
+    out.dim = dim_rr + 1;
     att = att / (1.0f - q);
   }
-  out.dim = halton.dim;
   if (in.bounce + 1 >= S.max_bounces) return out;
 
   out.alive = true;
diff --git a/platinum_amd/csrc/shade.hip b/platinum_amd/csrc/shade.hip
--- /dev/null
+++ b/platinum_amd/csrc/shade.hip
@@ -0,0 +1,270 @@
+#include <hip/hip_runtime.h>
+
+#include "kernels.h"
+#include "kernels_wave.h"
+#include "pt_shade.h"
+#include "queue_plan.h"
+
+namespace pt {
+
+#ifndef PT_SHADE_WAVES
+#define PT_SHADE_WAVES 5
+#endif
+#ifndef PT_SHADE_BLOCK
+#define PT_SHADE_BLOCK 256
+#endif
+constexpr uint32_t kShadeBlock = PT_SHADE_BLOCK;
+constexpr uint32_t kShadeHalton = 64;
+constexpr uint32_t kShadeLights = 8;
+constexpr int kLutE = 128, kLutEavg = 128, kLutEavgMs = 32;
+constexpr uint32_t kBinCap = 128;
+
+struct ShadeSlotIn : ShadeIn {
+  const vec4* q_rayO; const vec4* q_rayD; const vec4* q_hit;
+  const uint4* park;
+  const uint32_t* park_slot;
+};
+__device__ __forceinline__ uint32_t shade_lane() {
+  uint32_t t = threadIdx.x;
+  asm volatile("" : "+v"(t));
+  return t & 63u;
+}
+__device__ __forceinline__ uint4 parked(const ShadeSlotIn& in, uint32_t which) {
+  uint32_t t = threadIdx.x;
+  asm volatile("" : "+v"(t));
+  return in.park[which * kShadeBlock + t];
+}
+__device__ __forceinline__ vec3 path_att(const ShadeSlotIn& in) { const uint4 a = parked(in, 0); return v3(u2f(a.x), u2f(a.y), u2f(a.z)); }
+__device__ __forceinline__ uint32_t path_offset(const ShadeSlotIn& in) { return parked(in, 0).w; }
+__device__ __forceinline__ uint32_t path_dim(const ShadeSlotIn& in) { return (parked(in, 1).w & kMetaDimMask) + 1; }
+__device__ __forceinline__ LastRay path_last_ray(const ShadeSlotIn& in) {
+  uint32_t t = threadIdx.x;
+  asm volatile("" : "+v"(t));
+  const uint32_t i = in.park_slot[t];
+  const vec4 o4 = ldg(&in.q_rayO[i]), d4 = ldg(&in.q_rayD[i]), h4 = ldg(&in.q_hit[i]);
+  return {v3(o4.x, o4.y, o4.z), v3(d4.x, d4.y, d4.z), o4.w, h4.x, f2u(h4.w) & kHitTriMask, (f2u(d4.w) & kMetaSpecular) != 0};
+}
+
+__global__ void __launch_bounds__(PT_SHADE_BLOCK, (PT_SHADE_WAVES * 4 * 64) / PT_SHADE_BLOCK)
+k_shade(const DeviceScene* __restrict__ Sp, PathState sin, PathState sout, const vec4* __restrict__ hit, ShadowQueue sq,
+        vec4* __restrict__ Lbuf, Segments seg, uint32_t cur, BatchCounters* __restrict__ ctr, uint32_t bounce) {
+  PT_TAIL_BEGIN
+  const DeviceScene& S = *Sp;
+  __shared__ HaltonEntry lds_halton[kShadeHalton];
+  __shared__ LightRec lds_lights[kShadeLights];
+  __shared__ float lds_Eavg[kLutEavg];
+  __shared__ float lds_EavgMs[kLutEavgMs * kLutEavgMs];
+  static_assert(kMaxSegmentSlots <= 65536, "slot numbers inside a segment are binned as uint16_t (queue_plan.h bounds seg_cap)");
+  __shared__ uint16_t lds_bins[kShadeBlock / 64][5][kBinCap];
+  __shared__ uint32_t lds_bin_tri[kShadeBlock / 64][5][kBinCap];
+  __shared__ uint32_t lds_shadow_count[kShadeBlock / 64];
+  __shared__ uint32_t lds_park_slot[kShadeBlock];
+  __shared__ uint4 lds_park[2][kShadeBlock];
+  const uint32_t halton_base = 5u + 7u * bounce;
+  uint32_t halton_count = 11u + 5u * bounce;
+  if (halton_base >= (uint32_t)kHaltonDims) halton_count = 0;
+  else if (halton_base + halton_count > (uint32_t)kHaltonDims) halton_count = (uint32_t)kHaltonDims - halton_base;
+  if (halton_count > kShadeHalton) halton_count = kShadeHalton;
+  const bool lights_in_lds = S.lightCount <= kShadeLights;
+  {
+    const uint4* src = reinterpret_cast<const uint4*>(S.halton + halton_base);
+    uint4* dst = reinterpret_cast<uint4*>(lds_halton);
+    for (uint32_t i = threadIdx.x; i < halton_count * 2; i += kShadeBlock) dst[i] = ldg(&src[i]);
+    if (lights_in_lds) {
+      const uint4* ls = reinterpret_cast<const uint4*>(S.light_recs);
+      uint4* ld = reinterpret_cast<uint4*>(lds_lights);
+      for (uint32_t i = threadIdx.x; i < S.lightCount * (uint32_t)(sizeof(LightRec) / 16); i += kShadeBlock) ld[i] = ldg(&ls[i]);
+    }
+    for (uint32_t i = threadIdx.x; i < (uint32_t)kLutEavg; i += kShadeBlock) lds_Eavg[i] = ldg(&S.luts.Eavg.d[i]);
+    for (uint32_t i = threadIdx.x; i < (uint32_t)(kLutEavgMs * kLutEavgMs); i += kShadeBlock) lds_EavgMs[i] = ldg(&S.luts.EavgMs.d[i]);
+  }
+  __syncthreads();
+  ShadeTables T;
+  T.luts.E = Lut{S.luts.E.d, kLutE, kLutE, 1, 0};
+  T.luts.Eavg = Lut{lds_Eavg, kLutEavg, 1, 1, 1};
+  T.luts.EMs = Lut{S.luts.EMs.d, S.luts.EMs.w, S.luts.EMs.h, S.luts.EMs.depth, 0};
+  T.luts.EavgMs = Lut{lds_EavgMs, kLutEavgMs, kLutEavgMs, 1, 1};
+  T.luts.ETransIn = Lut{S.luts.ETransIn.d, S.luts.ETransIn.w, S.luts.ETransIn.h, S.luts.ETransIn.depth, 0};
+  T.luts.ETransOut = Lut{S.luts.ETransOut.d, S.luts.ETransOut.w, S.luts.ETransOut.h, S.luts.ETransOut.depth, 0};
+  T.halton = HaltonTab{S.halton, lds_halton, halton_base, halton_count};
+  T.lights = lights_in_lds ? lds_lights : S.light_recs;
+  T.light_cdf = S.light_cdf;
+  T.lights_lds = lights_in_lds ? 1 : 0;
+
+  uint32_t shaded = 0, total_out = 0, total_shadow = 0;
+  uint32_t claim = wave_index();
+  const uint32_t wave_in_block = __builtin_amdgcn_readfirstlane(threadIdx.x >> 6);
+  uint16_t* bin = &lds_bins[wave_in_block][0][0];
+  uint32_t* bin_tri = &lds_bin_tri[wave_in_block][0][0];
+  while (claim < seg.nseg) {
+    const uint32_t sg = __builtin_amdgcn_readfirstlane(seg.shade_order[claim]);
+    const unsigned long long seg_t0 = wall_clock64();
+    const uint32_t lbuf_base = segment_lbuf_base(seg, sg);
+    const uint32_t n = __builtin_amdgcn_readfirstlane(seg.active[cur][sg]);
+    uint32_t n_out = 0, n_shadow = 0;
+    const uint32_t seg_poisoned = S.env_texture < 0 ? __builtin_amdgcn_readfirstlane(seg.poison[sg]) : 0u;
+    unsigned long long poisoned_now = 0;
+    uint32_t cnt0 = 0, cnt1 = 0, cnt2 = 0, cnt3 = 0, cnt4 = 0;
+    uint32_t k0 = 0;
+    for (;;) {
+      const uint32_t lane = shade_lane();
+      while (k0 < n && cnt0 < 64 && cnt1 < 64 && cnt2 < 64 && cnt3 < 64 && cnt4 < 64) {
+        const uint32_t k = k0 + lane;
+        uint32_t cls = 5;
+        uint32_t w = 0;
+        if (k < n) {
+          w = f2u(hit[seg_slot(seg.nseg, sg, k)].w);
+          cls = w == kInvalidRef ? 4u : (w >> 28) & 3u;
+          if (w == kInvalidRef && S.env_texture < 0) {
+            if (!seg_poisoned) cls = 5u;
+            else {
+              const vec4 a4 = sin.att[seg_slot(seg.nseg, sg, k)];
+              if (!att_poisoned(v3(a4.x, a4.y, a4.z))) cls = 5u;
+            }
+          }
+        }
+        const unsigned long long m0 = __ballot(cls == 0), m1 = __ballot(cls == 1), m2 = __ballot(cls == 2), m3 = __ballot(cls == 3),
+                                 m4 = __ballot(cls == 4);
+        if (cls < 5) {
+          const uint32_t at = cls == 0 ? cnt0 + wave_prefix(m0) : cls == 1 ? cnt1 + wave_prefix(m1) : cls == 2 ? cnt2 + wave_prefix(m2)
+                            : cls == 3 ? cnt3 + wave_prefix(m3) : cnt4 + wave_prefix(m4);
+          bin[cls * kBinCap + at] = (uint16_t)k;
+          bin_tri[cls * kBinCap + at] = w & kHitTriMask;
+        }
+        cnt0 += (uint32_t)__popcll(m0); cnt1 += (uint32_t)__popcll(m1); cnt2 += (uint32_t)__popcll(m2);
+        cnt3 += (uint32_t)__popcll(m3); cnt4 += (uint32_t)__popcll(m4);
+        k0 += 64;
+      }
+      uint32_t k = kInvalidRef, tri = 0;
+      bool is_miss = false;
+      const uint32_t full = cnt0 >= 64 ? 0u : cnt1 >= 64 ? 1u : cnt2 >= 64 ? 2u : cnt3 >= 64 ? 3u : cnt4 >= 64 ? 4u : 5u;
+      if (full < 5) {
+        uint32_t c = 0;
+        if (full == 0) c = cnt0 -= 64; else if (full == 1) c = cnt1 -= 64; else if (full == 2) c = cnt2 -= 64;
+        else if (full == 3) c = cnt3 -= 64; else c = cnt4 -= 64;
+        k = bin[full * kBinCap + c + lane];
+        tri = bin_tri[full * kBinCap + c + lane];
+        is_miss = full == 4;
+      } else {
+        if (cnt0 + cnt1 + cnt2 + cnt3 + cnt4 == 0) break;
+        uint32_t taken = 0;
+#define PT_TAKE_FROM(c, cnt)                                                                                                   \
+        {                                                                                                                      \
+          const uint32_t take = cnt < 64 - taken ? cnt : 64 - taken;                                                           \
+          if (lane >= taken && lane < taken + take) { k = bin[c * kBinCap + cnt - take + (lane - taken)]; tri = bin_tri[c * kBinCap + cnt - take + (lane - taken)]; is_miss = c == 4; }  \
+          cnt -= take;                                                                                                         \
+          taken += take;                                                                                                       \
+        }
+        PT_TAKE_FROM(0, cnt0) PT_TAKE_FROM(1, cnt1) PT_TAKE_FROM(2, cnt2) PT_TAKE_FROM(3, cnt3) PT_TAKE_FROM(4, cnt4)
+#undef PT_TAKE_FROM
+      }
+      const bool has = k != kInvalidRef && !is_miss;
+      const uint32_t i = seg_slot(seg.nseg, sg, k != kInvalidRef ? k : 0u);
+      if (k != kInvalidRef && is_miss) {
+        const vec4 o4 = sin.rayO[i];
+        const vec4 d4 = sin.rayD[i];
+        const vec4 a4 = sin.att[i];
+        const vec3 att = v3(a4.x, a4.y, a4.z);
+        const uint32_t mpid = lbuf_base + (f2u(d4.w) >> kMetaPidShift);
+        vec4 L = Lbuf[mpid];
+        if (S.env_texture >= 0) {
+          const vec3 Le = stage_miss(S, v3(d4.x, d4.y, d4.z), att, bounce, o4.w, (f2u(d4.w) & kMetaSpecular) != 0);
+          L.x += Le.x; L.y += Le.y; L.z += Le.z;
+        }
+        L.x += att.x * 0.0f; L.y += att.y * 0.0f; L.z += att.z * 0.0f;
+        Lbuf[mpid] = L;
+      }
+      uint32_t c_alive = 0;
+      if (has) {
+        const vec4 h4 = ld_stream(&hit[i]);
+        const vec4 o4 = ld_stream(&sin.rayO[i]);
+        const vec4 d4 = ld_stream(&sin.rayD[i]);
+        const vec4 a4 = ld_stream(&sin.att[i]);
+        const uint32_t meta = f2u(d4.w);
+        ShadeSlotIn in;
+        in.o = v3(o4.x, o4.y, o4.z);
+        in.d = v3(d4.x, d4.y, d4.z);
+        in.q_rayO = sin.rayO; in.q_rayD = sin.rayD; in.q_hit = hit;
+        in.park = &lds_park[0][0];
+        in.park_slot = &lds_park_slot[0];
+        lds_park_slot[threadIdx.x] = i;
+        lds_park[0][threadIdx.x] = uint4{f2u(a4.x), f2u(a4.y), f2u(a4.z), f2u(a4.w)};
+        in.bounce = bounce;
+        in.t = h4.x; in.u = h4.y; in.v = h4.z;
+        in.tri = tri;
+        ShadeGeom g;
+        ShadingContext sc;
+        shade_geometry(S, in, g, sc);
+        lds_park[1][threadIdx.x] = uint4{f2u(g.hitPos.x), f2u(g.hitPos.y), f2u(g.hitPos.z), meta};
+        const BSDF bsdf(sc, S.flags, T.luts, g.wo);
+        uint32_t dim_rr;
+        {
+          const NeeOut nee = shade_nee(S, T, in, g, sc, bsdf, (meta & kMetaDimMask) + 1 + 6);
+          dim_rr = nee.dim;
+          const unsigned long long m = __ballot(nee.shadow);
+          if (nee.shadow) {
+            const uint32_t j = seg_slot(seg.nseg, sg, n_shadow + wave_prefix(m));
+            const uint4 hp = parked(in, 1);
+            st_stream(&sq.o[j], vec4{u2f(hp.x), u2f(hp.y), u2f(hp.z), nee.tmax});
+            st_stream(&sq.d[j], vec4{nee.d.x, nee.d.y, nee.d.z, u2f(lbuf_base + (hp.w >> kMetaPidShift))});
+            st_stream(&sq.contrib[j], vec4{nee.contrib.x, nee.contrib.y, nee.contrib.z, nee.payload});
+          }
+          lds_shadow_count[wave_in_block] = (uint32_t)__popcll(m);
+        }
+        const BounceOut bo = shade_bounce(S, T, in, g, sc, bsdf, dim_rr);
+        if (bo.has_emitted) {
+          const uint32_t pid = lbuf_base + (parked(in, 1).w >> kMetaPidShift);
+          vec4 L = Lbuf[pid];
+          L.x += bo.emitted.x; L.y += bo.emitted.y; L.z += bo.emitted.z;
+          Lbuf[pid] = L;
+        }
+        const unsigned long long m = __ballot(bo.alive);
+        poisoned_now |= __ballot(bo.alive && att_poisoned(bo.next_att));
+        if (bo.alive) {
+          const uint32_t j = seg_slot(seg.nseg, sg, n_out + wave_prefix(m));
+          const uint4 hp = parked(in, 1);
+          st_stream(&sout.rayO[j], vec4{u2f(hp.x), u2f(hp.y), u2f(hp.z), bo.next_pdf});
+          st_stream(&sout.rayD[j], vec4{bo.next_d.x, bo.next_d.y, bo.next_d.z, u2f((bo.dim & kMetaDimMask) | (bo.next_specular ? kMetaSpecular : 0u) | (hp.w & ~(kMetaDimMask | kMetaSpecular)))});
+          st_stream(&sout.att[j], vec4{bo.next_att.x, bo.next_att.y, bo.next_att.z, u2f(path_offset(in))});
+        }
+        c_alive = (uint32_t)__popcll(m);
+      }
+      const unsigned long long mh = __ballot(has);
+      if (mh) {
+        const int src = __builtin_ctzll(mh);
+        uint32_t z = 0;
+        asm volatile("" : "+v"(z));
+        n_shadow += __builtin_amdgcn_readfirstlane(lds_shadow_count[wave_in_block + z]);
+        n_out += (uint32_t)__builtin_amdgcn_readlane((int)c_alive, src);
+        shaded += (uint32_t)__popcll(mh);
+      }
+    }
+    if (shade_lane() == 0) {
+      seg.active[cur ^ 1][sg] = n_out;
+      seg.shadow[sg] = n_shadow;
+      if (poisoned_now) seg.poison[sg] = 1u;
+      seg.shade_cost[(size_t)bounce * seg.nseg + sg] = (uint32_t)(wall_clock64() - seg_t0) + 1u;
+    }
+    total_out += n_out;
+    total_shadow += n_shadow;
+    uint32_t next = 0;
+    if (shade_lane() == 0) next = wave_count() + atomicAdd(&ctr->work_shade[bounce], 1u);
+    claim = __builtin_amdgcn_readfirstlane(next);
+  }
+  if (shade_lane() == 0) {
+    WaveStats& ws = seg.stats[wave_index()];
+    ws.closest += total_out;
+    ws.shadow += total_shadow;
+    ws.shaded += shaded;
+  }
+  PT_TAIL_END(1)
+}
+
+uint32_t shade_block_threads() { return kShadeBlock; }
+uint32_t shade_blocks_per_cu() { return (PT_SHADE_WAVES * 4 * 64) / PT_SHADE_BLOCK; }
+void launch_shade(hipStream_t s, uint32_t grid, const DeviceScene* S, PathState sin, PathState sout, const vec4* hit,
+                  ShadowQueue sq, vec4* Lbuf, Segments seg, uint32_t cur, BatchCounters* ctr, uint32_t bounce) {
+  hipLaunchKernelGGL(k_shade, dim3(grid), dim3(kShadeBlock), 0, s, S, sin, sout, hit, sq, Lbuf, seg, cur, ctr, bounce);
+}
+
+}
```

Result: slower. 9260 Msamples/s (-2.5%).
